# vwxyzjn/cleanrl

Hardware: NVIDIA H100
Metric: env steps/sec (SPS) PPO Breakout num_envs=1024 (higher is better)
Workload: dtype bf16

## Files before the change

cleanrl_b200/_lib.py:

```python
from __future__ import annotations

import ctypes as C
from pathlib import Path

PKG = Path(__file__).resolve().parent
LIB_PATH = PKG / "libb200rl.so"

_p = C.c_void_p
_i64 = C.c_int64
_i = C.c_int
_d = C.c_double
_sz = C.c_size_t

SIGNATURES = {
    "b200rl_version": (_i, []),
    "b200rl_last_error": (C.c_char_p, []),
    "b200rl_compiled_arch": (_i, []),
    "b200rl_launch_count": (C.c_longlong, []),
    "b200rl_profile_enable": (None, [_i]),
    "b200rl_profile_reset": (None, []),
    "b200rl_profile_summary": (_i, [C.c_char_p, _sz]),
    "b200rl_gae_f32": (_i, [_p, _p, _p, _p, _p, _p, _p, _i64, _i64, _d, _d, _i, _p]),
    "b200rl_categorical_sample_f32": (_i, [_p, _i64, _p, _p, _i64, _i64, _i, _p, _p, _p, _p, _p]),
    "b200rl_categorical_eval_f32": (_i, [_p, _i64, _p, _i64, _i, _p, _p, _p]),
    "b200rl_ppo_loss_workspace_bytes": (_sz, [_i64]),
    "b200rl_ppo_loss_f32": (_i, [_p, _i64, _p, _i64, _p, _p, _p, _p, _p, _p, _i64, _i, _d, _d, _d, _i, _i,
                                 _p, _i64, _p, _i64, _p, _p, _sz, _p]),
    "b200rl_gaussian_sample_f32": (_i, [_p, _i64, _p, _p, _p, _i64, _i64, _i, _p, _p, _p, _p, _p]),
    "b200rl_gaussian_eval_f32": (_i, [_p, _i64, _p, _p, _i64, _i, _p, _p, _p]),
    "b200rl_ppo_loss_gaussian_workspace_bytes": (_sz, [_i64]),
    "b200rl_ppo_loss_gaussian_f32": (_i, [_p, _i64, _p, _p, _i64, _p, _p, _p, _p, _p, _p, _i64, _i, _d, _d, _d, _i, _i,
                                          _p, _i64, _p, _p, _i64, _p, _p, _sz, _p]),
    "b200rl_clip_adam_workspace_bytes": (_sz, [_i64]),
    "b200rl_clip_adam_f32": (_i, [_p, _p, _p, _p, _i64, _i64, _d, _d, _d, _d, _d, _i, _p, _p, _sz, _p]),
    "b200rl_adam_step_scalars": (_i, [_i64, _d, _d, _d, _p]),
    "b200rl_clip_adam_dyn_f32": (_i, [_p, _p, _p, _p, _i64, _p, _d, _d, _d, _d, _i, _p, _p, _sz, _p]),
    "b200rl_conv2d_fwd_f32": (_i, [_p, _i, _p, _d, _p, _p, _p, _i64, _i, _i, _i, _i, _i, _i, _i, _i, _p]),
    "b200rl_conv2d_bwd_data_f32": (_i, [_p, _p, _p, _i, _p, _i64, _i, _i, _i, _i, _i, _i, _i, _p]),
    "b200rl_conv2d_bwd_weight_workspace_bytes": (_sz, [_i64, _i, _i, _i, _i, _i, _i, _i]),
    "b200rl_conv2d_bwd_weight_f32": (_i, [_p, _i, _p, _d, _p, _p, _p, _i64, _i, _i, _i, _i, _i, _i, _i, _p, _sz, _p]),
    "b200rl_conv2d_fwd_pad_f32": (_i, [_p, _i, _p, _d, _p, _p, _p, _i64, _i, _i, _i, _i, _i, _i, _i, _i, _i, _p]),
    "b200rl_conv2d_bwd_data_pad_f32": (_i, [_p, _p, _p, _i, _p, _i64, _i, _i, _i, _i, _i, _i, _i, _i, _p]),
    "b200rl_conv2d_bwd_weight_pad_workspace_bytes": (_sz, [_i64, _i, _i, _i, _i, _i, _i, _i, _i]),
    "b200rl_conv2d_bwd_weight_pad_f32": (_i, [_p, _i, _p, _d, _p, _p, _p, _i64, _i, _i, _i, _i, _i, _i, _i, _i, _p, _sz, _p]),
    "b200rl_maxpool3s2_fwd_f32": (_i, [_p, _i64, _i, _i, _p, _p, _p]),
    "b200rl_maxpool3s2_bwd_f32": (_i, [_p, _p, _i64, _i, _i, _p, _p]),
    "b200rl_relu_f32": (_i, [_p, _i64, _p, _p]),
    "b200rl_relu_bwd_f32": (_i, [_p, _p, _p, _i64, _p, _p]),
    "b200rl_add_f32": (_i, [_p, _p, _i64, _p, _p]),
    "b200rl_nhwc_to_nchw_u8": (_i, [_p, _p, _i64, _i, _i, _i, _p, _p]),
    "b200rl_linear_fwd_f32": (_i, [_p, _p, _p, _p, _p, _i64, _i, _i, _i, _p]),
    "b200rl_linear_bwd_data_f32": (_i, [_p, _p, _p, _i, _p, _i64, _i, _i, _p]),
    "b200rl_linear_bwd_weight_workspace_bytes": (_sz, [_i64, _i, _i]),
    "b200rl_linear_bwd_weight_f32": (_i, [_p, _p, _p, _p, _p, _i64, _i, _i, _p, _sz, _p]),
    "b200rl_dqn_td_loss_workspace_bytes": (_sz, [_i64]),
    "b200rl_dqn_td_loss_f32": (_i, [_p, _i64, _p, _i64, _p, _p, _p, _i64, _i, _d, _i, _p, _i64, _p, _p, _sz, _p]),
    "b200rl_argmax_f32": (_i, [_p, _i64, _i64, _i, _p, _p]),
    "b200rl_c51_act_f32": (_i, [_p, _i64, _p, _i64, _i, _i, _p, _p, _p, _p, _p]),
    "b200rl_c51_loss_workspace_bytes": (_sz, [_i64]),
    "b200rl_c51_loss_f32": (_i, [_p, _i64, _p, _i64, _p, _p, _p, _p, _i64, _i, _i, _d, _d, _d, _p, _i64, _p, _p, _sz, _p]),
    "b200rl_naturecnn_param_count": (_i64, [_i]),
    "b200rl_naturecnn_bf16_packed_bytes": (_sz, [_i]),
    "b200rl_naturecnn_bf16_acts_bytes": (_sz, [_i64, _i]),
    "b200rl_frames_to_s2d_bf16": (_i, [_p, _p, _i64, _p, _p]),
    "b200rl_naturecnn_bf16_workspace_bytes": (_sz, [_i64, _i]),
    "b200rl_naturecnn_bf16_pack": (_i, [_p, _i, _p, _p]),
    "b200rl_naturecnn_bf16_forward": (_i, [_p, _i, _p, _i64, _i, _p, _p, _p, _p, _p]),
    "b200rl_naturecnn_bf16_backward": (_i, [_p, _p, _i, _p, _i64, _i, _p, _p, _p, _p, _p, _p, _sz, _p, _p]),
    "b200rl_frames_to_s2d_u8": (_i, [_p, _p, _i64, _p, _p, _p]),
    "b200rl_lstm_mask_state_f32": (_i, [_p, _p, _p, _i64, _i, _p, _p, _p]),
    "b200rl_lstm_cell_fwd_f32": (_i, [_p, _p, _p, _i64, _i, _p, _p, _p, _p]),
    "b200rl_lstm_cell_bwd_f32": (_i, [_p, _p, _p, _p, _p, _p, _p, _i64, _i, _p, _p, _p]),
    "b200rl_naturecnn_grad_tail_offset": (_i64, [_i]),
    "b200rl_frames_delta_s2d_u8": (_i, [_p, _p, _p, _p, _p, _i64, _p, _p, _p]),
    "b200rl_h2d_rows_async": (_i, [_p, _p, _i64, _i64, _i64, _p]),
    "b200rl_stackdelta_create": (_p, [_i64, _i, _i64, _i]),
    "b200rl_stackdelta_destroy": (None, [_p]),
    "b200rl_stackdelta_invalidate": (None, [_p]),
    "b200rl_stackdelta_begin": (_i64, [_p, _p, _i64, _p, _p, _p, _p]),
    "b200rl_stackdelta_wait": (_i64, [_p, _p]),
    "b200rl_mt19937_shuffle_i64": (_i, [_p, _p, _p, _i64]),
    "b200rl_stackdelta_launch": (_i64, [_p, _p, _i64, _p]),
    "b200rl_stackdelta_join": (_i64, [_p, _p, _p]),
    "b200rl_impala_param_count": (_i64, [_i]),
    "b200rl_impala_bf16_packed_bytes": (_sz, [_i]),
    "b200rl_impala_bf16_acts_bytes": (_sz, [_i64]),
    "b200rl_impala_bf16_acts_layout": (_i, [_i64, _p]),
    "b200rl_impala_bf16_workspace_bytes": (_sz, [_i64, _i]),
    "b200rl_impala_bf16_pack": (_i, [_p, _i, _p, _p]),
    "b200rl_impala_bf16_forward": (_i, [_p, _p, _i64, _i, _p, _p, _p, _p, _p]),
    "b200rl_impala_bf16_backward": (_i, [_p, _p, _i64, _i, _p, _p, _p, _p, _p, _p, _sz, _p]),
    "b200rl_impala_ppg_param_count": (_i64, [_i]),
    "b200rl_impala_ppg_bf16_packed_bytes": (_sz, [_i]),
    "b200rl_impala_ppg_bf16_workspace_bytes": (_sz, [_i64, _i]),
    "b200rl_impala_ppg_bf16_pack": (_i, [_p, _i, _p, _p]),
    "b200rl_impala_ppg_bf16_forward": (_i, [_p, _p, _i64, _i, _p, _p, _p, _p, _p]),
    "b200rl_impala_ppg_bf16_backward": (_i, [_p, _p, _i64, _i, _p, _p, _p, _p, _p, _p, _sz, _p]),
    "b200rl_clip_adam_ranges_f32": (_i, [_p, _p, _p, _p, _i64, _i64, _d, _p, _i, _i64, _d, _d, _d, _d, _d, _p, _p, _sz, _p]),
    "b200rl_clip_adam_ranges_dyn_f32": (_i, [_p, _p, _p, _p, _i64, _p, _p, _i, _i, _d, _d, _d, _d, _p, _p, _sz, _p]),
    "b200rl_ppg_aux_loss_workspace_bytes": (_sz, [_i64]),
    "b200rl_ppg_aux_loss_f32": (_i, [_p, _i64, _p, _p, _p, _i64, _i, _d, _d, _p, _i64, _p, _p, _sz, _p]),
    "b200rl_lstm_agent_param_count": (_i64, [_i]),
    "b200rl_lstm_agent_bf16_packed_bytes": (_sz, [_i]),
    "b200rl_lstm_agent_bf16_acts_bytes": (_sz, [_i64, _i64]),
    "b200rl_lstm_agent_bf16_acts_layout": (_i, [_i64, _i64, _p]),
    "b200rl_lstm_agent_bf16_workspace_bytes": (_sz, [_i64, _i64, _i]),
    "b200rl_lstm_agent_bf16_pack": (_i, [_p, _i, _p, _p]),
    "b200rl_lstm_agent_bf16_forward": (_i, [_p, _p, _i64, _i64, _i, _p, _p, _p, _p, _p, _p, _p, _p, _p, _p]),
    "b200rl_lstm_agent_bf16_backward": (_i, [_p, _p, _i64, _i64, _i, _p, _p, _p, _p, _p, _p, _p, _sz, _p]),
}



class PartLaunch(C.Structure):
    _fields_ = [("tracker", _p), ("copy_stream", _p), ("main_stream", _p), ("consumed_event", _p),
                ("n", C.c_int32), ("nchunks", C.c_int32), ("chunk_lo", C.c_int32 * 4), ("chunk_hi", C.c_int32 * 4),
                ("h2d_event", _p * 4), ("graph_exec", _p * 4),
                ("new_d", _p), ("slot_d", _p), ("full_d", _p), ("new_h", _p), ("full_h", _p), ("slot_h", _p),
                ("actions_d", _p), ("actions_h", _p), ("actions_bytes", _i64), ("d2h_event", _p)]


_lib = None


def load():
    global _lib
    if _lib is not None:
        return _lib
    if not LIB_PATH.exists():
        raise RuntimeError(
            f"{LIB_PATH} is missing: build it with `python -m cleanrl_b200.build` "
            "(the CUDA extension is the product; there is no CPU/torch fallback)")
    lib = C.CDLL(str(LIB_PATH))
    for name, (res, args) in SIGNATURES.items():
        fn = getattr(lib, name)
        fn.restype = res
        fn.argtypes = args
    _lib = lib
    return lib


def check(rc, what):
    if rc != 0:
        msg = load().b200rl_last_error().decode("utf-8", "replace")
        raise RuntimeError(f"libb200rl {what} failed (status {rc}): {msg}")
```

cleanrl_b200/agents.py:

```python
from __future__ import annotations

import numpy as np
import torch
import torch.nn as nn

from . import nets, ops


def layer_init(layer, std=np.sqrt(2), bias_const=0.0):
    torch.nn.init.orthogonal_(layer.weight, std)
    torch.nn.init.constant_(layer.bias, bias_const)
    return layer


def _exp_noise(n, A, device):
    return torch.empty(n, A, dtype=torch.float32, device=device).exponential_(1)


_exp_noise.graph_safe = True
_exp_noise.inplace = lambda buf: buf.exponential_(1)


class KernelAgent(nn.Module):

# ... 50 lines not shown

    @property
    def graph_friendly(self):
        return getattr(self.noise_fn, "graph_safe", False) and self.graph_capturable

    def noise_shape(self, n):
        return (n, self.num_actions)

    def draw_noise_into(self, buf):
        if hasattr(self.noise_fn, "inplace"):
            self.noise_fn.inplace(buf)
        else:
            buf.copy_(self.noise_fn(buf.shape[0], buf.shape[1], buf.device))

    def sample_into(self, obs, actions_out, logprobs_out, values_out, noise=None):
        logits, value = self._forward_heads(obs)
        n, A = logits.shape
        q = noise if noise is not None else self.noise_fn(n, A, logits.device)
        ops.categorical_sample(logits, q, value, out=(actions_out, logprobs_out, None, values_out))

    def loss_backward(self, policy_out, value, mb_inds, b, a, stats_row, scratch):
        M = policy_out.shape[0]
        if scratch.get("M") != M:
            scratch["M"] = M
            scratch["dhead"], scratch["dl"], scratch["dv"] = self.alloc_head_grad(M, policy_out.device)
        ops.ppo_loss(policy_out, value, mb_inds, b["actions"], b["logprobs"], b["advantages"], b["returns"], b["values"],
                     a.clip_coef, a.ent_coef, a.vf_coef, a.norm_adv, a.clip_vloss,
                     dlogits=scratch["dl"], dvalue=scratch["dv"], stats=stats_row)
        self.backward(scratch["dhead"])

    def alloc_head_grad(self, M, device):
        A = self.num_actions
        d = torch.empty(M, A + 1, dtype=torch.float32, device=device)
        return d, d[:, :A], d[:, A]

    def get_value(self, x):
        self.flat
        _, value = self._forward_heads(x)
        return value.reshape(-1, 1).clone() if not value.is_contiguous() else value.reshape(-1, 1)

    def get_action_and_value(self, x, action=None):
        self.flat
        logits, value = self._forward_heads(x)
        n, A = logits.shape
        if action is None:
            q = self.noise_fn(n, A, logits.device)
            action, logprob, entropy, v = ops.categorical_sample(logits, q, value)
        else:
            logprob, entropy = ops.categorical_eval(logits, action)
            v = value.clone() if not value.is_contiguous() else value
        return action, logprob, entropy, v.reshape(-1, 1)


class TensorCoreAgent(KernelAgent):

    precision = "fp32"
    plan_class = None
    _tc = None
    _tc_dirty = True

    def _head_outputs(self):
        return self.num_actions + 1

    def _plan_actions(self):
        return self._head_outputs() - 1

    def bind(self):
        self._tc, self._tc_dirty = None, True
        return super().bind()

    def uses_tc_plan(self):
        return self.precision == "bf16"

    @property
    def graph_capturable(self):
        return self.uses_tc_plan()

    def params_updated(self):
        self._tc_dirty = True

    def _tc_plan(self):
        f = self._flat
        if self._tc is None:
            self._tc = self.plan_class(self._plan_actions(), f.flat.device)
            assert f.flat.numel() >= self._tc.param_count
        if self._tc_dirty:
            self._tc.pack(f.flat)
            self._tc_dirty = False
        return self._tc

    def load_state_dict(self, *a, **k):
        out = super().load_state_dict(*a, **k)
        self._tc_dirty = True
        return out

    def pin_workspaces(self):
        if self._tc is not None:
            self._tc.pin()

    def _joint_head(self):
        f, A1, H = self._flat, self._head_outputs(), self.actor.in_features
        ow = (f.view_of(self.actor.weight)[0].data_ptr() - f.flat.data_ptr()) // 4
        ob = (f.view_of(self.actor.bias)[0].data_ptr() - f.flat.data_ptr()) // 4
        return nets.Linear(None, None, f.flat[ow:ow + A1 * H].view(A1, H), f.flat[ob:ob + A1],
                           f.grad[ow:ow + A1 * H].view(A1, H), f.grad[ob:ob + A1])


class NatureCNNAgent(TensorCoreAgent):

    plan_class = ops.NatureCNNBf16

    def __init__(self, envs):
        super().__init__()
        c, h, w = envs.single_observation_space.shape
        assert (c, h, w) == (4, 84, 84), "NatureCNN geometry is 4x84x84"
        trunk = []
        for cin, cout, k, s in ((4, 32, 8, 4), (32, 64, 4, 2), (64, 64, 3, 1)):
            trunk += [layer_init(nn.Conv2d(cin, cout, k, stride=s)), nn.ReLU()]
        trunk += [nn.Flatten(), layer_init(nn.Linear(64 * 7 * 7, 512)), nn.ReLU()]
        self.network = nn.Sequential(*trunk)
        self.actor = layer_init(nn.Linear(512, envs.single_action_space.n), std=0.01)
        self.critic = layer_init(nn.Linear(512, 1), std=1)
        self.num_actions = int(envs.single_action_space.n)

    def _param_order(self):
        net = [p for m in self.network for p in m.parameters()]
        return net + [self.actor.weight, self.critic.weight, self.actor.bias, self.critic.bias]

    def _build_plan(self):
        n = self.network
        self.trunk = nets.Chain([
            nets.Conv(n[0], "relu", in_div=255.0), nets.Conv(n[2], "relu"), nets.Conv(n[4], "relu"),
            nets.Linear(n[7], "relu")])
        self.head = self._joint_head()

    def _forward_heads(self, x, rows=None, keep=False, aux=None):
        if self.precision == "bf16":
            if x.dtype not in (torch.uint8, torch.bfloat16):
                x = x.to(torch.uint8)
            tc = self._tc_plan()
            out = tc.forward(x.contiguous(), rows, self._flat.flat)
            if keep:
                self._tc_obs, self._tc_rows, self._tc_aux = x, rows, aux
            A = self.num_actions
            return out[:, :A], out[:, A]
        if x.dtype not in (torch.uint8, torch.float32):
            x = x.float()
        hidden = self.trunk.fwd(x.contiguous(), rows=rows, keep=keep)
        out = self.head.fwd(hidden)
        if keep:
            self._hidden = hidden
        A = self.num_actions
        return out[:, :A], out[:, A]

    def forward_train(self, b_obs, mb_inds, aux=None):
        self.flat
        return self._forward_heads(b_obs, rows=mb_inds, keep=True, aux=aux)

    def grad_tail(self):
        if self.precision != "bf16":
            return None
        if getattr(self, "_tail_event", None) is None:
            self._tail_event = torch.cuda.Event()
            self._tail_event.record()
        return self._tc_plan().grad_tail_offset(), self._tail_event

    def backward(self, dhead):
        if self.precision == "bf16":
            self._tc.backward(self._tc_obs, self._tc_rows, self._flat.flat, dhead, self._flat.grad,
                              tail_event=getattr(self, "_tail_event", None), obs_aux=getattr(self, "_tc_aux", None))
            self._tc_obs = self._tc_rows = self._tc_aux = None
            return
        hidden = self._hidden
        self.head.bwd_weight(hidden, dhead)
        dh = self.head.bwd_data(dhead, hidden, "relu")
        self.trunk.bwd(dh)
        self._hidden = None


class MLPAgent(KernelAgent):

    def __init__(self, envs):
        super().__init__()
        d = int(np.array(envs.single_observation_space.shape).prod())
        A = int(envs.single_action_space.n)
        self.critic = nn.Sequential(layer_init(nn.Linear(d, 64)), nn.Tanh(), layer_init(nn.Linear(64, 64)), nn.Tanh(),
                                    layer_init(nn.Linear(64, 1), std=1.0))
        self.actor = nn.Sequential(layer_init(nn.Linear(d, 64)), nn.Tanh(), layer_init(nn.Linear(64, 64)), nn.Tanh(),
                                   layer_init(nn.Linear(64, A), std=0.01))
        self.num_actions = A

    def _build_plan(self):
        mk = lambda seq: nets.Chain([nets.Linear(seq[0], "tanh"), nets.Linear(seq[2], "tanh"), nets.Linear(seq[4], None)])
        self.c_chain, self.a_chain = mk(self.critic), mk(self.actor)

    def _forward_heads(self, x, rows=None, keep=False):
        x = x.float() if x.dtype != torch.float32 else x
        x = x.reshape(x.shape[0], -1).contiguous()
        logits = self.a_chain.fwd(x, rows=rows, keep=keep)
        value = self.c_chain.fwd(x, rows=rows, keep=keep)
        return logits, value[:, 0]

    def forward_train(self, b_obs, mb_inds):
        self.flat
        return self._forward_heads(b_obs, rows=mb_inds, keep=True)

    def alloc_head_grad(self, M, device):
        dl = torch.empty(M, self.num_actions, dtype=torch.float32, device=device)
        dv = torch.empty(M, 1, dtype=torch.float32, device=device)
        return (dl, dv), dl, dv[:, 0]

    def backward(self, dhead):
        dl, dv = dhead
        self.a_chain.bwd(dl)
        self.c_chain.bwd(dv)


class LSTMAgent(TensorCoreAgent):

    plan_class = ops.LSTMAgentBf16
    graph_capturable = False

    def __init__(self, envs):
        super().__init__()
        c, h, w = envs.single_observation_space.shape
        assert (h, w) == (84, 84), "NatureCNN trunk geometry is 84x84"
        trunk = []
        for cin, cout, k, s in ((c, 32, 8, 4), (32, 64, 4, 2), (64, 64, 3, 1)):
            trunk += [layer_init(nn.Conv2d(cin, cout, k, stride=s)), nn.ReLU()]
        trunk += [nn.Flatten(), layer_init(nn.Linear(64 * 7 * 7, 512)), nn.ReLU()]
        self.network = nn.Sequential(*trunk)
        self.lstm = nn.LSTM(512, 128)
        for name, param in self.lstm.named_parameters():
            if "bias" in name:
                nn.init.constant_(param, 0)
            elif "weight" in name:
                nn.init.orthogonal_(param, 1.0)
        self.actor = layer_init(nn.Linear(128, envs.single_action_space.n), std=0.01)
        self.critic = layer_init(nn.Linear(128, 1), std=1)
        self.num_actions = int(envs.single_action_space.n)
        self.hidden_size = 128

    def _param_order(self):
        net = [p for m in self.network for p in m.parameters()]
        return net + list(self.lstm.parameters()) + [self.actor.weight, self.critic.weight, self.actor.bias, self.critic.bias]

    def _build_plan(self):
        n = self.network
        self.trunk = nets.Chain([nets.Conv(n[0], "relu", in_div=255.0), nets.Conv(n[2], "relu"), nets.Conv(n[4], "relu"),
                                 nets.Linear(n[7], "relu")])
        self.head = self._joint_head()
        L = self.lstm
        self.l_ih = nets.Linear(None, None, L.weight_ih_l0.data, L.bias_ih_l0.data, L.weight_ih_l0.grad, L.bias_ih_l0.grad)
        self.l_hh = nets.Linear(None, None, L.weight_hh_l0.data, L.bias_hh_l0.data, L.weight_hh_l0.grad, L.bias_hh_l0.grad)

    def _tc_states(self, x, lstm_state, done, rows, keep):
        ops.LSTMAgentBf16.check_obs(x)
        H = self.hidden_size
        h0 = lstm_state[0].reshape(-1, H).to(torch.float32).contiguous()
        c0 = lstm_state[1].reshape(-1, H).to(torch.float32).contiguous()
        n = h0.shape[0]
        total = rows.numel() if rows is not None else x.shape[0]
        assert total % n == 0, "the sequence batch must be steps x envs"
        S = total // n
        done = done.reshape(-1).to(torch.float32).contiguous()
        x = x.contiguous()
        tc = self._tc_plan()
        self._tc_head, h, c = tc.forward(x, rows, S, n, self._flat.flat, h0, c0, done)
        if keep:
            self._tc_seq = (x, rows, S, n, done)
        return tc.act_tensors(S, n)["hseq"], (h.view(1, n, H), c.view(1, n, H))

    def get_states(self, x, lstm_state, done, rows=None, keep=False):
        self.flat
        if self.precision == "bf16":
            return self._tc_states(x, lstm_state, done, rows, keep)
        H = self.hidden_size
        h, c = lstm_state[0].reshape(-1, H).contiguous(), lstm_state[1].reshape(-1, H).contiguous()
        n = h.shape[0]
        if x.dtype not in (torch.uint8, torch.float32):
            x = x.float()
        feats = self.trunk.fwd(x.contiguous(), rows=rows, keep=keep)
        total = feats.shape[0]
        assert total % n == 0, "the sequence batch must be steps x envs"
        S = total // n
        dev = feats.device
        done = done.reshape(S, n).to(torch.float32).contiguous()
        gx = self.l_ih.fwd(feats)
        hidden = torch.empty(S, n, H, dtype=torch.float32, device=dev)
        hm = torch.empty(S, n, H, dtype=torch.float32, device=dev)
        cm = torch.empty(S, n, H, dtype=torch.float32, device=dev)
        save = torch.empty(S, n, 5 * H, dtype=torch.float32, device=dev) if keep else None
        c_cur = torch.empty(n, H, dtype=torch.float32, device=dev)
        for t in range(S):
            ops.lstm_mask_state(h, c, done[t], out=(hm[t], cm[t]))
            gh = self.l_hh.fwd(hm[t])
            ops.lstm_cell_fwd(gx[t * n:(t + 1) * n], gh, cm[t], hidden[t], c_cur, save[t] if keep else None)
            h, c = hidden[t], c_cur
            if t + 1 < S:
                c_cur = torch.empty(n, H, dtype=torch.float32, device=dev)
        if keep:
            self._seq = dict(feats=feats, hidden=hidden, hm=hm, cm=cm, save=save, done=done, S=S, n=n)
        return hidden.view(S * n, H), (h.reshape(1, n, H).clone(), c.reshape(1, n, H).clone())

    def _heads(self, hidden):
        out = self._tc_head if self.precision == "bf16" else self.head.fwd(hidden)
# ... 480 lines not shown
```

cleanrl_b200/csrc/net_tc.cu:

```cuda
#include <cuda.h>
#include <algorithm>
#include "tc_base.cuh"
#include "tc_conv_win.cuh"
#include "tc_conv1_u8.cuh"
#include "tc_gemm_tma.cuh"
#include "tc_wgrad_win.cuh"
#include "tc_reduce.cuh"
#include "tc_aux.cuh"
#include "tc_heads.cuh"
#include "tc_heads_wide.cuh"
#include "tc_lstm.cuh"

namespace b200rl {

struct NatureLayout {
    int A;
    int64_t c1w, c1b, c2w, c2b, c3w, c3b, fcw, fcb, hw, hb, total;
    int64_t w1f, w2f, w2dg, w3f, w3dg, wfcf, wfcdg, w1l, w1sc, packed_total;
    bool wide; int G; int64_t whf, whdg, hbp;
    int64_t wih, whh, bih, bhh, whhp;
    explicit NatureLayout(int A_) : A(A_), wih(-1), whh(-1), bih(-1), bhh(-1), whhp(-1) {
        int64_t o = 0;
        c1w = o; o += 32 * 4 * 8 * 8;  c1b = o; o += 32;
        c2w = o; o += 64 * 32 * 4 * 4; c2b = o; o += 64;
// ... 16 lines not shown
        G = wide ? (int)ceil_div(A + 1, kWideHeadPad) * kWideHeadPad : 0;
        whf = whdg = hbp = 0;
        if (wide) {
            whf = q; q += (int64_t)G * 512;
            whdg = q; q += (int64_t)G * 512;
            hbp = q; q += (int64_t)G * 2;
        }
        packed_total = q;
    }
    struct Lstm {};
    NatureLayout(int A_, Lstm) : A(A_) {
        int64_t o = 0;
        c1w = o; o += 32 * 8 * 8;      c1b = o; o += 32;
        c2w = o; o += 64 * 32 * 4 * 4; c2b = o; o += 64;
        c3w = o; o += 64 * 64 * 3 * 3; c3b = o; o += 64;
        fcw = o; o += 512 * 3136;      fcb = o; o += 512;
        wih = o; o += 512 * 512;       whh = o; o += 512 * 128;
        bih = o; o += 512;             bhh = o; o += 512;
        hw = o;  o += (int64_t)(A + 1) * 128;
        hb = o;  o += A + 1;
        total = o;
        int64_t q = 0;
        w1f = q; q += 32 * 64;
        w2f = q; q += 64 * 512;
        w2dg = q; q += 4 * 32 * 256;
        w3f = q; q += 64 * 576;
        w3dg = q; q += 64 * 576;
        wfcf = q; q += 512 * 3136;
        wfcdg = q; q += 3136 * 512;
        w1l = w1sc = -1;
        wide = true; G = 512;
        whf = q; q += 512 * 512;
        whdg = q; q += 512 * 512;
        hbp = q; q += 512 * 2;
        whhp = q; q += 512 * 128;
        packed_total = q;
    }
};

struct NatureActs {
    int64_t x0, act1, act2, act3, hid, dhid, dact3a, dact3b, dact2a, dact2b, dact1, m1, m2, m3, m4, total;
    explicit NatureActs(int64_t n, bool with_x0 = true) {
        int64_t o = 0;
        x0 = o; if (with_x0) o += n * 28224;
        act1 = o; o += n * 12800;
        act2 = o; o += n * 5184;
        act3 = o; o += n * 3136;
        hid = o;  o += n * 512;
        dhid = o; o += n * 512;
        dact3a = o; o += n * 5184;
        dact3b = o; o += n * 7744;
        dact2a = o; o += n * 6400;
        dact2b = o; o += n * 7744;
        dact1 = o; o += n * 14112;
        auto pad8 = [](int64_t v) { return (v + 7) & ~int64_t(7); };
        m1 = o; o += pad8(n * 100 * 4 * 2);
        m2 = o; o += pad8(n * 81 * 2 * 2);
        m3 = o; o += pad8(n * 49 * 2 * 2);
        m4 = o; o += pad8(n * 16 * 2);
        total = o;
    }
};

static void gemm_rowmajor(KGemmParams& p, const bf16* x, int64_t n, int nchunks) {
    memset(&p, 0, sizeof(p));
    p.scale = 1.f;
    p.A = x; p.M = n; p.nchunks = nchunks;
}


static void win_defaults(WinParams& p) { memset(&p, 0, sizeof(p)); p.scale = 1.f; }
static int round8(int v) { return (v + 7) & ~7; }
static void win_conv1(WinParams& p, const bf16* x0, const int64_t* rows, int64_t n) {
    p.A = x0; p.rows = rows; p.n = (int)n; p.G = 441; p.Wp = 21; p.M = n * 441;
    p.tpi_shift = 2;
    p.n_images = rows ? (int64_t)1 << 24 : n;
    p.ntaps = 4; p.shift[0] = 0; p.shift[1] = 1; p.shift[2] = 21; p.shift[3] = 22; p.WR = round8(128 + 22);
}
static void win_conv2(WinParams& p, const bf16* act1, int64_t n) {
    p.A = act1; p.n = (int)n; p.G = 100; p.Wp = 10; p.M = n * 100;
    p.ntaps = 4; p.shift[0] = 0; p.shift[1] = 1; p.shift[2] = 10; p.shift[3] = 11; p.WR = round8(128 + 11);
}
static void win_conv3(WinParams& p, const bf16* act2, int64_t n) {
    p.A = act2; p.n = (int)n; p.G = 81; p.Wp = 9; p.M = n * 81;
    p.ntaps = 9; for (int ky = 0; ky < 3; ++ky) for (int kx = 0; kx < 3; ++kx) p.shift[ky * 3 + kx] = ky * 9 + kx;
    p.WR = round8(128 + 20);
}
static void wgw_defaults(WGradWinParams& w) { memset(&w, 0, sizeof(w)); }

static const int kC1Ctas = 264, kC2Ctas = 132, kC3Ctas = 132;
static WPlan conv1_wgrad_plan(int64_t n, bool u8) {
    return u8 ? wgrad_plan(n * 512, kC2Ctas, 512) : wgrad_plan(n * 512, kC1Ctas, 128);
}
static WPlan conv2_wgrad_plan(int64_t n) { return wgrad_plan(n * 100, kC2Ctas, 128); }
static WPlan conv3_wgrad_plan(int64_t n) { return wgrad_plan(n * 81, kC3Ctas, 128); }

static size_t wgrad_win_bytes(int splits, int nslots) { return (size_t)splits * nslots * 64 * 64 * sizeof(float); }
static size_t wgrad_win_bias_bytes(int splits) { return (size_t)splits * 64 * sizeof(float); }
static int launch_wgrad_win(const WGradWinParams& p, int ctas, cudaStream_t s, const char* what) {
    const size_t smem = (size_t)kWgradWinStages * ((size_t)p.WRX * 128 * p.cpr + 128 * 128) + 4096 + 1024;
    static SmemAttrCache attr;
    if (int rc0 = attr.ensure(tc_wgrad_win, smem, what)) return rc0;
    CUtensorMap tmX, tmY;
    memset(&tmX, 0, sizeof(tmX)); memset(&tmY, 0, sizeof(tmY));
    const int use_tma = p.tpi_shift ? 0 : 1;
    if (p.rows_per_cta % 128 != 0) return fail(B200RL_ERR_INVALID_ARGUMENT, "%s: rows per CTA must be a multiple of 128", what);
    if (ctas < 1 || (int64_t)(ctas - 1) * p.rows_per_cta >= p.M)
        return fail(B200RL_ERR_INVALID_ARGUMENT, "%s: every row split must own at least one row", what);
    int rc;
    if (use_tma) {
        if (p.rows || p.ldy != 64 || p.ncolsY != 64)
            return fail(B200RL_ERR_INVALID_ARGUMENT, "%s: linear-grid mode needs contiguous rows and 64-channel dY", what);
        if ((rc = make_tmap_2d(&tmX, p.X, p.M, (int64_t)p.cpr * 64, p.WRX, what))) return rc;
        if ((rc = make_tmap_2d(&tmY, p.Y, p.M, 64, 128, what))) return rc;
    } else {
        if ((128 << p.tpi_shift) < p.G) return fail(B200RL_ERR_INVALID_ARGUMENT, "%s: steps per image too small", what);
        if ((rc = make_tmap_3d(&tmX, p.X, p.n_images, p.G, (int64_t)p.cpr * 64, p.WRX, what))) return rc;
    }
    const dim3 grid((unsigned)ceil_div(p.nslots / 2, kWgradWinTilesPerCta), ctas);
    tc_wgrad_win<<<grid, kWgradWinThreads, smem, s>>>(tmX, tmY, p, use_tma);
    return check_launch(what);
}

}

using namespace b200rl;

namespace b200rl {
static bool head_ok(int A) { return A >= 1 && A < kMaxWideHeads; }
static size_t wide_dhead_bytes(int64_t n, const NatureLayout& L) { return ((size_t)n * L.G * 2 + 255) & ~(size_t)255; }
static size_t wide_small_bytes(int64_t n, const NatureLayout& L, int A1) {
    return wide_dhead_bytes(n, L) + colsum_f32_ws(n, A1);
}

static int trunk_fwd(const NatureLayout& L, const NatureActs& Q, const float* params, const bf16* P, bf16* act, int64_t n,
                     cudaStream_t s) {
    int rc;
    KGemmParams p;
    WinParams wp;
    win_defaults(wp); win_conv2(wp, act + Q.act1, n);
    wp.Bw = P + L.w2f; wp.N = 64; wp.vH = 9; wp.vW = 9; wp.out_mode = WOUT_DENSE; wp.out = act + Q.act2;
    wp.bias = params + L.c2b; wp.relu = 1; wp.mask_out = reinterpret_cast<uint32_t*>(act + Q.m2);
    { ProfScope ps(s, "conv2_fwd", 2.0 * n * 81 * 64 * 512, (double)n * ((12800 + 5184) * 2 + 648));
      if ((rc = launch_conv_win_t<128, 2, 2, 4>(wp, s, "naturecnn/conv2"))) return rc; }
    win_defaults(wp); win_conv3(wp, act + Q.act2, n);
    wp.Bw = P + L.w3f; wp.N = 64; wp.vH = 7; wp.vW = 7; wp.out_mode = WOUT_DENSE; wp.out = act + Q.act3;
    wp.bias = params + L.c3b; wp.relu = 1; wp.mask_out = reinterpret_cast<uint32_t*>(act + Q.m3);
    { ProfScope ps(s, "conv3_fwd", 2.0 * n * 49 * 64 * 576, (double)n * ((5184 + 3136) * 2 + 392));
      if ((rc = launch_conv_win_t<128, 1, 4, 9>(wp, s, "naturecnn/conv3"))) return rc; }
    gemm_rowmajor(p, act + Q.act3, n, 49);
    p.Bw = P + L.wfcf; p.N = 512; p.out = act + Q.hid; p.ldo = 512; p.bias = params + L.fcb; p.relu = 1;
    p.mask_out = reinterpret_cast<uint32_t*>(act + Q.m4);
    { ProfScope ps(s, "fc_fwd", 2.0 * n * 512 * 3136, (double)n * (3136 + 512) * 2 + 512.0 * 3136 * 2);
      if (n <= 8192) { if ((rc = launch_gemm_tma<64, 6>(p, s, "naturecnn/fc"))) return rc; }
      else if ((rc = launch_gemm_tma<128, 4>(p, s, "naturecnn/fc"))) return rc; }
    return B200RL_OK;
}

static int trunk_bwd(const NatureLayout& L, const NatureActs& Q, const bf16* P, bf16* act, float* grads, int64_t n,
                     float* wsbig, float* wssmall, void* tail_ready_event, bool dact1_fused, cudaStream_t s) {
    int rc;
    KGemmParams p;
    {
        int splits;
        { ProfScope ps(s, "fc_wgrad", 2.0 * n * 512 * 3136, (double)n * (3136 + 512) * 2 + 512.0 * 3136 * 4);
          if ((splits = launch_wgrad_tma(act + Q.dhid, 512, act + Q.act3, 3136, n, wsbig, s, "naturecnn/fc_wgrad")) < 0) return splits; }
        { ProfScope ps(s, "wgrad_fold_bias", 0, 0);
          note_launches(1); tc_fold_fc<<<(unsigned)ceil_div((int64_t)512 * 3136, 256), 256, 0, s>>>(wsbig, splits, 512, 13 * 256, 512, 3136, 64, 49, 1.f, grads + L.fcw);
          if ((rc = colsum(act + Q.dhid, n, 512, 512, wssmall, grads + L.fcb, s))) return rc; }
        if (tail_ready_event) {
            cudaError_t e = cudaEventRecord(reinterpret_cast<cudaEvent_t>(tail_ready_event), s);
            if (e != cudaSuccess) return fail(B200RL_ERR_CUDA, "naturecnn_backward: cudaEventRecord: %s", cudaGetErrorString(e));
        }
        gemm_rowmajor(p, act + Q.dhid, n, 8);
        p.Bw = P + L.wfcdg; p.N = 3136; p.out = act + Q.dact3a; p.out2 = act + Q.dact3b; p.dual_dact3 = 1;
        p.ldo = 3136; p.mask_bits = reinterpret_cast<const uint32_t*>(act + Q.m3);
        { ProfScope ps(s, "fc_dgrad", 2.0 * n * 512 * 3136, (double)n * ((3136 + 512) * 2 + 392) + 512.0 * 3136 * 2);
          if ((rc = launch_gemm_tma<128, 4>(p, s, "naturecnn/fc_dgrad"))) return rc; }
    }
    WGradWinParams gw;
    WinParams wp;
    FoldWin fw;
    {
        wgw_defaults(gw);
        gw.X = act + Q.act2; gw.M = n * 81; gw.n = (int)n; gw.G = 81; gw.cpr = 1; gw.nslots = 10; gw.WRX = round8(128 + 20);
        for (int t = 0; t < 9; ++t) gw.shift[t] = (t / 3) * 9 + (t % 3);
        const int st[10] = {0, 1, 2, 3, 4, 5, 6, 7, 7, 8};
        for (int k = 0; k < 10; ++k) { gw.slot_tap[k] = st[k]; gw.slot_cc[k] = 0; }
        gw.Y = act + Q.dact3a; gw.ldy = 64; gw.ncolsY = 64;
        const WPlan pl = conv3_wgrad_plan(n);
        gw.rows_per_cta = pl.rows_per_cta; gw.ws = wsbig; gw.wsb = wssmall;
        { ProfScope ps(s, "conv3_wgrad", 2.0 * n * 49 * 64 * 576, (double)n * (5184 + 5184) * 2);
          if ((rc = launch_wgrad_win(gw, pl.splits, s, "naturecnn/conv3_wgrad"))) return rc; }
        memset(&fw, 0, sizeof(fw));
        fw.layer = 3; fw.S = pl.splits; fw.nslots = 10; fw.Cout = 64; fw.scale = 1.f; fw.bscale = 1.f;
        for (int k = 0; k < 10; ++k) { fw.slot_tap[k] = st[k]; fw.slot_skip[k] = (k == 8); }
        { ProfScope ps(s, "wgrad_fold_bias", 0, 0);
          fw.wsb = wssmall; fw.db = grads + L.c3b;
          tc_fold_win<<<(unsigned)ceil_div(640 * 64 + 64, 32), 256, 0, s>>>(wsbig, fw, grads + L.c3w);
          if ((rc = check_launch("naturecnn/conv3_fold"))) return rc; }
        win_defaults(wp);
        wp.A = act + Q.dact3b; wp.n = (int)n; wp.G = 121; wp.Wp = 11; wp.M = n * 121; wp.ntaps = 9;
        for (int ky = 0; ky < 3; ++ky) for (int kx = 0; kx < 3; ++kx) wp.shift[ky * 3 + kx] = (2 - ky) * 11 + (2 - kx);
        wp.WR = round8(128 + 24);
        wp.Bw = P + L.w3dg; wp.N = 64; wp.vH = 9; wp.vW = 9; wp.out_mode = WOUT_DACT2;
        wp.out = act + Q.dact2a; wp.out2 = act + Q.dact2b; wp.mask_bits = reinterpret_cast<const uint32_t*>(act + Q.m2);
        { ProfScope ps(s, "conv3_dgrad", 2.0 * n * 81 * 64 * 576, (double)n * ((7744 + 6400 + 7744) * 2 + 648));
          if ((rc = launch_conv_win_t<128, 1, 4, 9>(wp, s, "naturecnn/conv3_dgrad"))) return rc; }
    }
    {
        wgw_defaults(gw);
        gw.X = act + Q.act1; gw.M = n * 100; gw.n = (int)n; gw.G = 100; gw.cpr = 2; gw.nslots = 8; gw.WRX = round8(128 + 11);
        gw.shift[0] = 0; gw.shift[1] = 1; gw.shift[2] = 10; gw.shift[3] = 11;
        for (int k = 0; k < 8; ++k) { gw.slot_tap[k] = k >> 1; gw.slot_cc[k] = k & 1; }
        gw.Y = act + Q.dact2a; gw.ldy = 64; gw.ncolsY = 64;
        const WPlan pl = conv2_wgrad_plan(n);
        gw.rows_per_cta = pl.rows_per_cta; gw.ws = wsbig; gw.wsb = wssmall;
        { ProfScope ps(s, "conv2_wgrad", 2.0 * n * 81 * 64 * 512, (double)n * (12800 + 6400) * 2);
          if ((rc = launch_wgrad_win(gw, pl.splits, s, "naturecnn/conv2_wgrad"))) return rc; }
        memset(&fw, 0, sizeof(fw));
        fw.layer = 2; fw.S = pl.splits; fw.nslots = 8; fw.Cout = 64; fw.scale = 1.f; fw.bscale = 1.f;
        for (int k = 0; k < 8; ++k) { fw.slot_tap[k] = k >> 1; fw.slot_cc[k] = k & 1; }
        { ProfScope ps(s, "wgrad_fold_bias", 0, 0);
          fw.wsb = wssmall; fw.db = grads + L.c2b;
          tc_fold_win<<<(unsigned)ceil_div(512 * 64 + 64, 32), 256, 0, s>>>(wsbig, fw, grads + L.c2w);
          if ((rc = check_launch("naturecnn/conv2_fold"))) return rc; }
        if (dact1_fused) return B200RL_OK;
        win_defaults(wp);
        wp.A = act + Q.dact2b; wp.n = (int)n; wp.G = 121; wp.Wp = 11; wp.M = n * 121; wp.ntaps = 4;
        for (int a = 0; a < 2; ++a) for (int b = 0; b < 2; ++b) wp.shift[a * 2 + b] = (1 - a) * 11 + (1 - b);
        wp.WR = round8(128 + 12);
        wp.Bw = P + L.w2dg; wp.N = 128; wp.vH = 10; wp.vW = 10; wp.out_mode = WOUT_DACT1;
        wp.out = act + Q.dact1; wp.mask_bits = reinterpret_cast<const uint32_t*>(act + Q.m1);
        { ProfScope ps(s, "conv2_dgrad", 2.0 * n * 400 * 32 * 256, (double)n * ((7744 + 14112) * 2 + 1600));
          if ((rc = launch_conv_win<128, 1, 4, 4>(wp, s, "naturecnn/conv2_dgrad"))) return rc; }
    }
    return B200RL_OK;
}
static size_t trunk_big_bytes(int64_t n) {
    return std::max({wgrad_tma_bytes(n, 512, 3136), wgrad_win_bytes(conv3_wgrad_plan(n).splits, 10),
                     wgrad_win_bytes(conv2_wgrad_plan(n).splits, 8)});
}
static size_t trunk_small_bytes(int64_t n) {
    return std::max({colsum_ws(n, 512), wgrad_win_bias_bytes(conv3_wgrad_plan(n).splits),
                     wgrad_win_bias_bytes(conv2_wgrad_plan(n).splits)});
}

static int wide_head_fwd(const NatureLayout& L, const bf16* P, const bf16* hid, int64_t n, int A1, float* out, cudaStream_t s) {
    KGemmParams p;
    gemm_rowmajor(p, hid, n, 8);
    p.Bw = P + L.whf; p.N = L.G; p.bias = reinterpret_cast<const float*>(P + L.hbp);
    p.out_f32 = out; p.ldo = A1; p.ncols_f32 = A1;
    return launch_gemm_tma<128, 4>(p, s, "wide_heads");
}

static int wide_head_bwd(const NatureLayout& L, const bf16* P, const float* dhead, int64_t n, int A1, const bf16* hid, bf16* dhid,
                         const uint32_t* hid_bits, float* dW, float* db, float* wsbig, float* wssmall, cudaStream_t s) {
    int rc;
    KGemmParams p;
    bf16* dh16 = reinterpret_cast<bf16*>(wssmall);
    float* dbpart = reinterpret_cast<float*>(reinterpret_cast<char*>(wssmall) + wide_dhead_bytes(n, L));
    int cb = (int)ceil_div(n * L.G, 256); if (cb > num_sms() * 8) cb = num_sms() * 8;
    tc_head_dhead_bf16<<<cb, 256, 0, s>>>(dhead, n, A1, L.G, dh16);
    if ((rc = check_launch("wide_heads_dhead"))) return rc;
    if ((rc = colsum_f32(dhead, n, A1, dbpart, db, s))) return rc;
    const int splits = launch_wgrad_tma(dh16, L.G, hid, 512, n, wsbig, s, "wide_heads_wgrad");
    if (splits < 0) return splits;
    tc_fold_fc<<<(unsigned)ceil_div((int64_t)A1 * 512, 256), 256, 0, s>>>(wsbig, splits, L.G, 512, A1, 512, 512, 1, 1.f, dW);
    if ((rc = check_launch("wide_heads_wgrad"))) return rc;
    gemm_rowmajor(p, dh16, n, L.G / 64);
    p.Bw = P + L.whdg; p.N = 512; p.out = dhid; p.ldo = 512;
    p.mask_bits = hid_bits;
    if (n <= 8192) { if ((rc = launch_gemm_tma<64, 6>(p, s, "wide_heads_dgrad"))) return rc; }
    else if ((rc = launch_gemm_tma<128, 4>(p, s, "wide_heads_dgrad"))) return rc;
    return B200RL_OK;
}
}

extern "C" int64_t b200rl_naturecnn_param_count(int A) { return A >= 1 ? NatureLayout(A).total : -1; }
extern "C" int64_t b200rl_naturecnn_grad_tail_offset(int A) { return A >= 1 ? NatureLayout(A).fcw : -1; }
extern "C" size_t b200rl_naturecnn_bf16_packed_bytes(int A) { return head_ok(A) ? (size_t)NatureLayout(A).packed_total * 2 : 0; }
extern "C" size_t b200rl_naturecnn_bf16_acts_bytes(int64_t n, int obs_format) {
    return n >= 0 ? (size_t)NatureActs(n, obs_format == B200RL_OBS_U8_NCHW).total * 2 + 256 : 0;
}

extern "C" int b200rl_frames_to_s2d_bf16(const uint8_t* obs, const int64_t* rows, int64_t n, void* out, void* stream) {
    B200RL_REQUIRE(n >= 0, "frames_to_s2d: negative n");
    if (n == 0) return B200RL_OK;
    B200RL_REQUIRE(obs && out, "frames_to_s2d: null pointer");
    B200RL_REQUIRE(aligned(obs, 4) && aligned(out, 16), "frames_to_s2d: misaligned buffer");
    cudaStream_t s = (cudaStream_t)stream;
    ProfScope ps(s, "frames_to_s2d", 0, (double)n * 28224 * 3);
    tc_frames_to_s2d<<<(unsigned)ceil_div(n * 1764, 256), 256, 0, s>>>(obs, rows, n, reinterpret_cast<bf16*>(out));
    return check_launch("frames_to_s2d");
}

extern "C" int b200rl_frames_to_s2d_u8(const uint8_t* obs, const int64_t* rows, int64_t n, uint8_t* out_rm, uint8_t* out_cm, void* stream) {
    B200RL_REQUIRE(n >= 0, "frames_to_s2d_u8: negative n");
    if (n == 0) return B200RL_OK;
    B200RL_REQUIRE(obs && out_rm && out_cm, "frames_to_s2d_u8: null pointer");
    B200RL_REQUIRE(aligned(obs, 16) && aligned(out_rm, 16) && aligned(out_cm, 16), "frames_to_s2d_u8: misaligned buffer");
    B200RL_REQUIRE(n <= (int64_t)1 << 28, "frames_to_s2d_u8: n too large");
    cudaStream_t s = (cudaStream_t)stream;
    ProfScope ps(s, "frames_to_s2d", 0, (double)n * (28224 + 28224 + 28672));
    tc_frames_to_s2d_u8<<<(unsigned)(n * 4), 256, 0, s>>>(obs, rows, n, out_rm, out_cm);
    return check_launch("frames_to_s2d_u8");
}

static size_t naturecnn_big_bytes(int64_t n, const NatureLayout& L) {
    return std::max({trunk_big_bytes(n), L.wide ? wgrad_tma_bytes(n, L.G, 512) : 0,
                     wgrad_win_bytes(conv1_wgrad_plan(n, false).splits, 4), wgrad_win_bytes(conv1_wgrad_plan(n, true).splits, 4)});
}

extern "C" size_t b200rl_naturecnn_bf16_workspace_bytes(int64_t n, int A) {
    if (n < 1 || !head_ok(A)) return 0;
    const NatureLayout L(A);
    const size_t small = std::max({trunk_small_bytes(n), L.wide ? wide_small_bytes(n, L, A + 1) : heads_partial_bytes(n, A + 1, 512),
                                   wgrad_win_bias_bytes(conv1_wgrad_plan(n, false).splits),
                                   wgrad_win_bias_bytes(conv1_wgrad_plan(n, true).splits)});
    return naturecnn_big_bytes(n, L) + small + 512;
}

extern "C" int b200rl_naturecnn_bf16_pack(const float* params, int A, void* packed, void* stream) {
    B200RL_REQUIRE(params && packed && head_ok(A), "naturecnn_pack: bad arguments (A must be in [1,%d])", kMaxWideHeads - 1);
    B200RL_REQUIRE(aligned(packed, 16), "naturecnn_pack: packed buffer must be 16-B aligned");
    const NatureLayout L(A);
    bf16* P = reinterpret_cast<bf16*>(packed);
    cudaStream_t s = (cudaStream_t)stream;
    ProfScope ps(s, "pack_weights", 0, (double)L.total * 4 + (double)L.packed_total * 2);
    tc_pack_conv1_s2d<<<32, 256, 0, s>>>(params + L.c1w, P + L.w1f);
    tc_pack_conv1_i8<<<32, 256, 0, s>>>(params + L.c1w, reinterpret_cast<int8_t*>(P + L.w1l), reinterpret_cast<float*>(P + L.w1sc));
    tc_pack_conv2_cells<<<128, 256, 0, s>>>(params + L.c2w, P + L.w2f);
    tc_pack_conv_s2_classes<<<(unsigned)ceil_div(32768, 256), 256, 0, s>>>(params + L.c2w, 64, 32, P + L.w2dg);
    tc_pack_conv<<<(unsigned)ceil_div(36864, 256), 256, 0, s>>>(params + L.c3w, 64, 64, 3, 3, 0, P + L.w3f, P + L.w3dg);
    tc_pack_fc<<<dim3(512 / 8, 49 / 7), 256, 0, s>>>(params + L.fcw, 512, 49, P + L.wfcf, P + L.wfcdg);
    if (L.wide) {
        tc_pack_head_wide<<<(unsigned)ceil_div((int64_t)L.G * 512, 256), 256, 0, s>>>(params + L.hw, params + L.hb, A + 1, L.G,
                                                                                    P + L.whf, P + L.whdg, reinterpret_cast<float*>(P + L.hbp));
        return check_launch("naturecnn_pack", 7);
    }
    return check_launch("naturecnn_pack", 6);
}

extern "C" int b200rl_naturecnn_bf16_forward(const void* obs, int obs_format, const int64_t* rows, int64_t n, int A,
                                             const float* params, const void* packed, void* acts,
                                             float* head_out, void* stream) {
    B200RL_REQUIRE(n >= 0, "naturecnn_forward: negative n");
    if (n == 0) return B200RL_OK;
    B200RL_REQUIRE(obs && params && packed && acts && head_out, "naturecnn_forward: null pointer");
    B200RL_REQUIRE(head_ok(A), "naturecnn_forward: A=%d outside [1,%d]", A, kMaxWideHeads - 1);
    B200RL_REQUIRE(obs_format == B200RL_OBS_U8_NCHW || obs_format == B200RL_OBS_S2D_BF16 || obs_format == B200RL_OBS_S2D_U8,
                   "naturecnn_forward: bad obs_format %d", obs_format);
    B200RL_REQUIRE(aligned(obs, 16) && aligned(acts, 16) && aligned(packed, 16), "naturecnn_forward: misaligned buffer");
    B200RL_REQUIRE(n <= (int64_t)1 << 22, "naturecnn_forward: n too large");
    const NatureLayout L(A);
    const NatureActs Q(n, obs_format == B200RL_OBS_U8_NCHW);
    const bf16* P = reinterpret_cast<const bf16*>(packed);
    bf16* act = reinterpret_cast<bf16*>(acts);
    cudaStream_t s = (cudaStream_t)stream;
    int rc;
    WinParams wp;
    const bf16* x0 = reinterpret_cast<const bf16*>(obs);
    const int64_t* x0rows = rows;
    if (obs_format == B200RL_OBS_U8_NCHW) {
        if ((rc = b200rl_frames_to_s2d_bf16(reinterpret_cast<const uint8_t*>(obs), rows, n, act + Q.x0, stream))) return rc;
        x0 = act + Q.x0; x0rows = nullptr;
    }
    if (obs_format == B200RL_OBS_S2D_U8) {
        Conv1U8Params cp;
        memset(&cp, 0, sizeof(cp));
        cp.rows = rows; cp.n = (int)n; cp.n_images = rows ? (int64_t)1 << 24 : n;
        cp.limbs = reinterpret_cast<const int8_t*>(P + L.w1l); cp.sc = reinterpret_cast<const float*>(P + L.w1sc);
        cp.bias = params + L.c1b; cp.out = act + Q.act1; cp.mask_out = reinterpret_cast<uint32_t*>(act + Q.m1);
        ProfScope ps(s, "conv1_fwd", 2.0 * n * 400 * 32 * 256, (double)n * (28224 + 12800 * 2 + 1600));
        if ((rc = launch_conv1_i8(cp, obs, s, "naturecnn/conv1_i8"))) return rc;
    } else {
    win_defaults(wp); win_conv1(wp, x0, x0rows, n);
    wp.Bw = P + L.w1f; wp.N = 32; wp.vH = 20; wp.vW = 20; wp.out_mode = WOUT_S2D2; wp.out = act + Q.act1;
    wp.bias = params + L.c1b; wp.scale = 1.0f / 255.0f; wp.relu = 1; wp.mask_out = reinterpret_cast<uint32_t*>(act + Q.m1);
    { ProfScope ps(s, "conv1_fwd", 2.0 * n * 400 * 32 * 256, (double)n * ((28224 + 12800) * 2 + 1600));
      if ((rc = launch_conv_win<32, 1, 9, 4>(wp, s, "naturecnn/conv1"))) return rc; }
    }
    if ((rc = trunk_fwd(L, Q, params, P, act, n, s))) return rc;
    if (L.wide) {
        ProfScope ps(s, "heads_fwd", 2.0 * n * 512 * (A + 1), (double)n * (1024 + 4 * (A + 1)) + (double)L.G * 1024);
        return wide_head_fwd(L, P, act + Q.hid, n, A + 1, head_out, s);
    }
    ProfScope ps(s, "heads_fwd", 2.0 * n * 512 * (A + 1), (double)n * (1024 + 4 * (A + 1)));
    return heads_fwd<512>(act + Q.hid, params + L.hw, params + L.hb, n, A + 1, head_out, s, "naturecnn/heads");
}

extern "C" int b200rl_naturecnn_bf16_backward(const void* obs, const void* obs_aux, int obs_format, const int64_t* rows, int64_t n, int A,
                                              const float* params, const void* packed, void* acts,
                                              const float* dhead, float* grads,
                                              void* workspace, size_t workspace_bytes, void* tail_ready_event, void* stream) {
    B200RL_REQUIRE(n >= 1, "naturecnn_backward: n must be >= 1");
    B200RL_REQUIRE(obs && params && packed && acts && dhead && grads && workspace, "naturecnn_backward: null pointer");
    B200RL_REQUIRE(head_ok(A), "naturecnn_backward: A=%d outside [1,%d]", A, kMaxWideHeads - 1);
    B200RL_REQUIRE(aligned(workspace, 16), "naturecnn_backward: workspace misaligned");
    const size_t need = b200rl_naturecnn_bf16_workspace_bytes(n, A);
    if (workspace_bytes < need) return fail(B200RL_ERR_WORKSPACE, "naturecnn_backward: workspace %zu < %zu", workspace_bytes, need);
    B200RL_REQUIRE(obs_format == B200RL_OBS_U8_NCHW || obs_format == B200RL_OBS_S2D_BF16 || obs_format == B200RL_OBS_S2D_U8,
                   "naturecnn_backward: bad obs_format %d", obs_format);
    B200RL_REQUIRE(obs_format != B200RL_OBS_S2D_U8 || (obs_aux && aligned(obs_aux, 16)), "naturecnn_backward: the uint8 rollout needs obs_aux");
    const NatureLayout L(A);
    const NatureActs Q(n, obs_format == B200RL_OBS_U8_NCHW);
    const bf16* P = reinterpret_cast<const bf16*>(packed);
    bf16* act = reinterpret_cast<bf16*>(acts);
    cudaStream_t s = (cudaStream_t)stream;
    const bf16* x0 = obs_format == B200RL_OBS_U8_NCHW ? act + Q.x0 : reinterpret_cast<const bf16*>(obs);
    const int64_t* x0rows = obs_format == B200RL_OBS_U8_NCHW ? nullptr : rows;
    const size_t big = (naturecnn_big_bytes(n, L) + 255) & ~(size_t)255;
    float* wsbig = reinterpret_cast<float*>(workspace);
    float* wssmall = reinterpret_cast<float*>(reinterpret_cast<char*>(workspace) + big);
    int rc;
    const int A1 = A + 1;
    if (L.wide) {
        ProfScope ps(s, "heads_bwd", 4.0 * n * 512 * A1, (double)n * (2048 + 64 + 8 * A1));
        if ((rc = wide_head_bwd(L, P, dhead, n, A1, act + Q.hid, act + Q.dhid, reinterpret_cast<const uint32_t*>(act + Q.m4),
                                grads + L.hw, grads + L.hb, wsbig, wssmall, s))) return rc;
    } else
    {
        ProfScope ps(s, "heads_bwd", 4.0 * n * 512 * A1, (double)n * (2048 + 64 + 8 * A1));
        if ((rc = heads_bwd_weight<512>(dhead, act + Q.hid, n, A1, wssmall, grads + L.hw, grads + L.hb, s, "naturecnn/heads_bwd"))) return rc;
        if ((rc = heads_bwd_data<512>(dhead, params + L.hw, reinterpret_cast<const uint8_t*>(act + Q.m4), n, A1, act + Q.dhid, s,
                                      "naturecnn/heads_bwd"))) return rc;
    }
    if ((rc = trunk_bwd(L, Q, P, act, grads, n, wsbig, wssmall, tail_ready_event, obs_format == B200RL_OBS_S2D_U8, s))) return rc;
    const bool u8 = obs_format == B200RL_OBS_S2D_U8;
    const WPlan pl = conv1_wgrad_plan(n, u8);
    if (u8) {
        Conv21BwdU8Params cw;
        memset(&cw, 0, sizeof(cw));
        cw.rows = rows; cw.n = (int)n; cw.rows_per_cta = pl.rows_per_cta; cw.ws = wsbig; cw.wsb = wssmall;
        cw.w2dg = P + L.w2dg; cw.m1 = reinterpret_cast<const uint32_t*>(act + Q.m1);
        { ProfScope ps(s, "conv21_bwd", 2.0 * 2.0 * n * 400 * 32 * 256, (double)n * (7744 * 2 + 1600 + 28672 + 14112 * 2));
          if ((rc = launch_conv21_bwd_u8(cw, obs_aux, rows ? (int64_t)1 << 24 : n, act + Q.dact2b, act + Q.dact1, pl.splits, s,
                                         "naturecnn/conv21_bwd_u8"))) return rc; }
    } else {
        WGradWinParams gw;
        wgw_defaults(gw);
        gw.X = x0; gw.rows = x0rows; gw.M = n * 512; gw.n = (int)n; gw.G = 441; gw.cpr = 1; gw.nslots = 4; gw.WRX = round8(128 + 22);
        gw.tpi_shift = 2; gw.n_images = x0rows ? (int64_t)1 << 24 : n;
        gw.shift[0] = 0; gw.shift[1] = 1; gw.shift[2] = 21; gw.shift[3] = 22;
        for (int k = 0; k < 4; ++k) { gw.slot_tap[k] = k; gw.slot_cc[k] = 0; }
        gw.Y = act + Q.dact1; gw.ldy = 32; gw.ncolsY = 32;
        gw.rows_per_cta = pl.rows_per_cta; gw.ws = wsbig; gw.wsb = wssmall;
        { ProfScope ps(s, "conv1_wgrad", 2.0 * n * 400 * 32 * 256, (double)n * (28224 + 14112) * 2);
          if ((rc = launch_wgrad_win(gw, pl.splits, s, "naturecnn/conv1_wgrad"))) return rc; }
    }
    FoldWin fw;
    memset(&fw, 0, sizeof(fw));
    fw.layer = 1; fw.S = pl.splits; fw.nslots = 4; fw.Cout = 32;
    fw.scale = u8 ? 1.0f / 255.0f / kDact1Scale : 1.0f / 255.0f;
    fw.bscale = u8 ? 1.0f / kDact1Scale : 1.f;
    for (int k = 0; k < 4; ++k) fw.slot_tap[k] = k;
    { ProfScope ps(s, "wgrad_fold_bias", 0, 0);
      fw.wsb = wssmall; fw.db = grads + L.c1b;
      tc_fold_win<<<(unsigned)ceil_div(256 * 32 + 32, 32), 256, 0, s>>>(wsbig, fw, grads + L.c1w);
      if ((rc = check_launch("naturecnn/conv1_fold"))) return rc; }
    return B200RL_OK;
}

namespace b200rl {
constexpr int64_t kLstmMaxRows = (int64_t)1 << 17;

struct LstmActs {
    NatureActs T;
    int64_t gx, hseq, hm, save, cm, dgates, total;
    explicit LstmActs(int64_t M) : T(M, false) {
        int64_t o = (T.total * 2 + 255) & ~int64_t(255);
        auto take = [&](int64_t bytes) { const int64_t r = o; o += (bytes + 255) & ~int64_t(255); return r; };
        gx = take(M * 512 * 4);
        hseq = take(M * 128 * 2);
        hm = take(M * 128 * 2);
        save = take(M * 640 * 4);
        cm = take(M * 128 * 4);
        dgates = take(M * 512 * 4);
        total = o;
    }
};

static bool lstm_heads_ok(int A) { return A >= 1 && A + 1 <= lstm::kMaxA1; }
static bool lstm_sizes_ok(int64_t S, int64_t n) { return S >= 1 && n >= 1 && S <= kLstmMaxRows && n <= kLstmMaxRows && S * n <= kLstmMaxRows; }

struct C1Plan { int64_t per_cta; int ctas; };
static C1Plan lstm_conv1_plan(int64_t M) {
    C1Plan c;
    const int64_t want = M < kC1Ctas ? M : kC1Ctas;
    c.per_cta = ceil_div(M, want);
    c.ctas = (int)ceil_div(M, c.per_cta);
    return c;
}
static size_t lstm_big_bytes(int64_t M, const NatureLayout& L) {
    const size_t a = std::max({wgrad_tma_bytes(M, L.G, 512), wgrad_tma_bytes(M, 512, 128), trunk_big_bytes(M),
                               (size_t)lstm_conv1_plan(M).ctas * 32 * 64 * 4});
    return (a + 255) & ~(size_t)255;
}
static size_t lstm_small_bytes(int64_t M, const NatureLayout& L) {
    return std::max({heads_partial_bytes(M, L.A + 1, 128), wide_small_bytes(M, L, 512), trunk_small_bytes(M),
                     (size_t)lstm_conv1_plan(M).ctas * 32 * 4});
}
}

extern "C" int64_t b200rl_lstm_agent_param_count(int A) { return A >= 1 ? NatureLayout(A, NatureLayout::Lstm{}).total : -1; }
extern "C" size_t b200rl_lstm_agent_bf16_packed_bytes(int A) {
    return lstm_heads_ok(A) ? (size_t)NatureLayout(A, NatureLayout::Lstm{}).packed_total * 2 : 0;
}
extern "C" size_t b200rl_lstm_agent_bf16_acts_bytes(int64_t S, int64_t n) {
    return lstm_sizes_ok(S, n) ? (size_t)LstmActs(S * n).total : 0;
}
extern "C" int b200rl_lstm_agent_bf16_acts_layout(int64_t S, int64_t n, int64_t* offsets) {
    B200RL_REQUIRE(offsets, "lstm_acts_layout: null pointer");
    B200RL_REQUIRE(lstm_sizes_ok(S, n), "lstm_acts_layout: S=%lld n=%lld out of range", (long long)S, (long long)n);
    const LstmActs Q(S * n);
    const int64_t v[B200RL_LSTM_ACTS_TENSORS] = {Q.T.act1 * 2, Q.T.m1 * 2, Q.T.act2 * 2, Q.T.act3 * 2, Q.T.hid * 2, Q.T.m4 * 2,
                                                 Q.gx, Q.hseq, Q.hm, Q.save, Q.cm, Q.dgates, Q.T.dhid * 2};
    for (int k = 0; k < B200RL_LSTM_ACTS_TENSORS; ++k) offsets[k] = v[k];
    return B200RL_OK;
}
extern "C" size_t b200rl_lstm_agent_bf16_workspace_bytes(int64_t S, int64_t n, int A) {
    if (!lstm_sizes_ok(S, n) || !lstm_heads_ok(A)) return 0;
    const NatureLayout L(A, NatureLayout::Lstm{});
    return lstm_big_bytes(S * n, L) + lstm_small_bytes(S * n, L) + 512;
}

extern "C" int b200rl_lstm_agent_bf16_pack(const float* params, int A, void* packed, void* stream) {
    B200RL_REQUIRE(params && packed, "lstm_pack: null pointer");
    B200RL_REQUIRE(lstm_heads_ok(A), "lstm_pack: A=%d outside [1,%d]", A, lstm::kMaxA1 - 1);
    B200RL_REQUIRE(aligned(params, 16) && aligned(packed, 16), "lstm_pack: misaligned buffer");
    const NatureLayout L(A, NatureLayout::Lstm{});
    bf16* P = reinterpret_cast<bf16*>(packed);
    cudaStream_t s = (cudaStream_t)stream;
    ProfScope ps(s, "pack_weights", 0, (double)L.total * 4 + (double)L.packed_total * 2);
    lstm::lstm_pack_conv1<<<8, 256, 0, s>>>(params + L.c1w, P + L.w1f);
    tc_pack_conv2_cells<<<128, 256, 0, s>>>(params + L.c2w, P + L.w2f);
    tc_pack_conv_s2_classes<<<(unsigned)ceil_div(32768, 256), 256, 0, s>>>(params + L.c2w, 64, 32, P + L.w2dg);
    tc_pack_conv<<<(unsigned)ceil_div(36864, 256), 256, 0, s>>>(params + L.c3w, 64, 64, 3, 3, 0, P + L.w3f, P + L.w3dg);
    tc_pack_fc<<<dim3(512 / 8, 49 / 7), 256, 0, s>>>(params + L.fcw, 512, 49, P + L.wfcf, P + L.wfcdg);
    tc_pack_head_wide<<<(unsigned)ceil_div((int64_t)L.G * 512, 256), 256, 0, s>>>(params + L.wih, params + L.bih, 512, L.G,
                                                                                P + L.whf, P + L.whdg, reinterpret_cast<float*>(P + L.hbp));
    tc_head_dhead_bf16<<<256, 256, 0, s>>>(params + L.whh, 512, 128, 128, P + L.whhp);
// ... 122 lines not shown
```

cleanrl_b200/csrc/policy.cu:

```cuda
#include "common.cuh"
#include <cfloat>

namespace b200rl {

constexpr int kMaxA = 64;

struct RowStats {
    float lse;
    float m2;
    float s2;
};

__device__ __forceinline__ RowStats row_stats(const float* __restrict__ x, int A) {
    float m = -INFINITY;
    for (int k = 0; k < A; ++k) m = fmaxf(m, x[k]);
    const float mm = (fabsf(m) == INFINITY) ? 0.f : m;
    float s = 0.f;
    for (int k = 0; k < A; ++k) s += expf(x[k] - mm);
    RowStats r;
    r.lse = logf(s) + mm;
    float m2 = -INFINITY;
    for (int k = 0; k < A; ++k) m2 = fmaxf(m2, x[k] - r.lse);
    float s2 = 0.f;
    for (int k = 0; k < A; ++k) s2 += expf((x[k] - r.lse) - m2);
    r.m2 = m2;
    r.s2 = s2;
    return r;
}

__global__ void __launch_bounds__(128) categorical_sample_kernel(
    const float* __restrict__ logits, int64_t ld, const float* __restrict__ noise,
    const float* __restrict__ value_in, int64_t ldv, int64_t n, int A,
    int64_t* __restrict__ action, float* __restrict__ logprob, float* __restrict__ entropy,
    float* __restrict__ value_out) {
    const int64_t i = (int64_t)blockIdx.x * blockDim.x + threadIdx.x;
    if (i >= n) return;
    const float* x = logits + i * ld;
    const float* q = noise + i * (int64_t)A;
    const RowStats rs = row_stats(x, A);
    float best = -INFINITY, ent = 0.f;
    int arg = 0;
    for (int k = 0; k < A; ++k) {
        const float nl = x[k] - rs.lse;
        const float p = expf(nl - rs.m2) / rs.s2;
        const float sc = p / q[k];
        if (sc > best) { best = sc; arg = k; }
        ent += fmaxf(nl, -FLT_MAX) * p;
    }
    action[i] = arg;
    logprob[i] = x[arg] - rs.lse;
    if (entropy) entropy[i] = -ent;
    if (value_out && value_in) value_out[i] = value_in[i * ldv];
}

__global__ void __launch_bounds__(128) categorical_eval_kernel(
    const float* __restrict__ logits, int64_t ld, const int64_t* __restrict__ action, int64_t n, int A,
    float* __restrict__ logprob, float* __restrict__ entropy) {
    const int64_t i = (int64_t)blockIdx.x * blockDim.x + threadIdx.x;
    if (i >= n) return;
    const float* x = logits + i * ld;
    const RowStats rs = row_stats(x, A);
    float ent = 0.f;
    for (int k = 0; k < A; ++k) {
        const float nl = x[k] - rs.lse;
        ent += fmaxf(nl, -FLT_MAX) * (expf(nl - rs.m2) / rs.s2);
    }
    int a = (int)action[i];
    a = a < 0 ? 0 : (a >= A ? A - 1 : a);
    logprob[i] = x[a] - rs.lse;
    if (entropy) entropy[i] = -ent;
}

__device__ __forceinline__ float adv_pass(const float* __restrict__ b_adv, const int64_t* __restrict__ inds, int64_t M,
                                          float mean, bool squared) {
    float s = 0.f;
    const int64_t step = blockDim.x;
    int64_t i = threadIdx.x;
    for (; i + 7 * step < M; i += 8 * step) {
        int64_t j[8];
        float v[8];
#pragma unroll
        for (int u = 0; u < 8; ++u) j[u] = inds ? __ldg(inds + i + u * step) : i + u * step;
#pragma unroll
        for (int u = 0; u < 8; ++u) v[u] = __ldg(b_adv + j[u]);
#pragma unroll
        for (int u = 0; u < 8; ++u) {
            const float d = v[u] - mean;
            s += squared ? d * d : v[u];
        }
    }
    for (; i < M; i += step) {
        const float v = b_adv[inds ? inds[i] : i];
        const float d = v - mean;
        s += squared ? d * d : v;
    }
    return s;
}
__global__ void __launch_bounds__(1024) adv_stats_kernel(
    const float* __restrict__ b_adv, const int64_t* __restrict__ inds, int64_t M, float* __restrict__ out2) {
    __shared__ float red[32];
    const float mean = block_sum(adv_pass(b_adv, inds, M, 0.f, false), red) / (float)M;
    const float ss = block_sum(adv_pass(b_adv, inds, M, mean, true), red);
    if (threadIdx.x == 0) {
        out2[0] = mean;
        out2[1] = sqrtf(ss / (float)(M - 1));
    }
}

constexpr int kLossThreads = 256;
constexpr int kNumStats = 7;

struct LossParams {
    const float* logits; int64_t ld;
    const float* value; int64_t ldv;
    const int64_t* inds;
    const int64_t* b_actions;
    const float* b_logprobs; const float* b_adv; const float* b_ret; const float* b_val;
    int64_t M; int A;
    float clip, ent_coef, vf_coef;
    int norm_adv, clip_vloss;
    float* dlogits; int64_t ldd;
    float* dvalue; int64_t lddv;
    float* stats;
    const float* adv_stats;
    float* partials;
    unsigned int* ticket;
};

__global__ void __launch_bounds__(kLossThreads) ppo_loss_kernel(LossParams P) {
    __shared__ float red[32];
    __shared__ bool is_last;
    const int64_t i = (int64_t)blockIdx.x * blockDim.x + threadIdx.x;
    float acc[kNumStats];
#pragma unroll
    for (int k = 0; k < kNumStats; ++k) acc[k] = 0.f;
    if (i < P.M) {
        const int64_t j = P.inds ? P.inds[i] : i;
        const float* x = P.logits + i * P.ld;
        const int A = P.A;
        const int a = (int)P.b_actions[j];
        const RowStats rs = row_stats(x, A);
        float ent = 0.f;
        for (int k = 0; k < A; ++k) {
            const float nl = x[k] - rs.lse;
            const float p = expf(nl - rs.m2) / rs.s2;
            ent += fmaxf(nl, -FLT_MAX) * p;
        }
        ent = -ent;
        const float newlogprob = x[a] - rs.lse;
        const float logratio = newlogprob - P.b_logprobs[j];
        const float ratio = expf(logratio);
        float adv = P.b_adv[j];
        if (P.norm_adv) adv = (adv - P.adv_stats[0]) / (P.adv_stats[1] + 1e-8f);
        const float lo = 1.f - P.clip, hi = 1.f + P.clip;
        const float rc = fminf(fmaxf(ratio, lo), hi);
        const float pg1 = -adv * ratio, pg2 = -adv * rc;
        const float pg = fmaxf(pg1, pg2);
        const float nv = P.value[i * P.ldv];
        const float R = P.b_ret[j], V = P.b_val[j];
        float vterm, gv;
        const float du = nv - R;
        const float vu = du * du;
        if (P.clip_vloss) {
            const float d = nv - V;
            const float vcl = V + fminf(fmaxf(d, -P.clip), P.clip);
            const float dc = vcl - R;
            const float vc = dc * dc;
            vterm = fmaxf(vu, vc);
            const float gu = 2.f * du;
            const float gc = (d >= -P.clip && d <= P.clip) ? 2.f * dc : 0.f;
            gv = (vu > vc) ? gu : ((vc > vu) ? gc : 0.5f * (gu + gc));
        } else {
            vterm = vu;
            gv = 2.f * du;
        }
        acc[0] = pg;
        acc[1] = vterm;
        acc[2] = ent;
        acc[3] = -logratio;
        acc[4] = (ratio - 1.f) - logratio;
        acc[5] = (fabsf(ratio - 1.0f) > P.clip) ? 1.f : 0.f;
        const float invM = 1.0f / (float)P.M;
        const float inrange = (ratio >= lo && ratio <= hi) ? 1.f : 0.f;
        float g_ratio = 0.f;
        if (pg1 > pg2) g_ratio = -adv;
        else if (pg1 == pg2) g_ratio = 0.5f * (-adv) * (1.f + inrange);
        const float g_lp = g_ratio * ratio * invM;
        const float g_ent = -P.ent_coef * invM;
        float* dl = P.dlogits + i * P.ldd;
        for (int k = 0; k < A; ++k) {
            const float nl = x[k] - rs.lse;
            const float p = expf(nl - rs.m2) / rs.s2;
            const float onehot = (k == a) ? 1.f : 0.f;
            dl[k] = g_lp * (onehot - p) + g_ent * (-p * (nl + ent));
        }
        P.dvalue[i * P.lddv] = P.vf_coef * 0.5f * invM * gv;
    }
#pragma unroll
    for (int k = 0; k < 6; ++k) {
        const float s = block_sum(acc[k], red);
        if (threadIdx.x == 0) P.partials[(int64_t)blockIdx.x * kNumStats + k] = s;
    }
    if (threadIdx.x == 0) {
        __threadfence();
// ... 364 lines not shown
```

cleanrl_b200/csrc/tc_conv1_u8.cuh:

```cuda
#pragma once
#include "tc_base.cuh"
#include <cuda_fp16.h>
#include "tc_conv_win.cuh"

namespace b200rl {
using namespace tc;

__device__ __forceinline__ uint64_t desc_kmajor_sw64(uint32_t smem_addr) {
    return (uint64_t)((smem_addr & 0x3FFFFu) >> 4) | (1ull << 16) | (32ull << 32) | kDescSwizzle64;
}
__device__ __forceinline__ uint64_t desc_mnmajor_sw64(uint32_t smem_addr, uint32_t lbo) {
    return (uint64_t)((smem_addr & 0x3FFFFu) >> 4) | ((uint64_t)((lbo >> 4) & 0x3FFF) << 16) | (32ull << 32) | kDescSwizzle64;
}
__device__ __forceinline__ uint32_t img64_off(int r, int c) { return (uint32_t)(r * 64 + ((c ^ ((r >> 1) & 3)) << 4)); }
__global__ void __launch_bounds__(256) tc_frames_to_s2d_u8(const uint8_t* __restrict__ obs, const int64_t* __restrict__ rows, int64_t n,
                                                           uint8_t* __restrict__ out_rm, uint8_t* __restrict__ out_cm) {
    __shared__ __align__(16) uint8_t plane[7056];
    const int64_t i = blockIdx.x >> 2;
    const int c = blockIdx.x & 3;
    const int64_t img = rows ? rows[i] : i;
    const int4* src = reinterpret_cast<const int4*>(obs + img * 28224 + c * 7056);
    for (int t = threadIdx.x; t < 441; t += 256) reinterpret_cast<int4*>(plane)[t] = __ldg(src + t);
    __syncthreads();
    for (int pos = threadIdx.x; pos < 441; pos += 256) {
        const int Y = pos / 21, X = pos - Y * 21;
        const uint8_t* p = plane + (Y * 4) * 84 + X * 4;
        int4 v;
        v.x = *reinterpret_cast<const int*>(p); v.y = *reinterpret_cast<const int*>(p + 84);
        v.z = *reinterpret_cast<const int*>(p + 168); v.w = *reinterpret_cast<const int*>(p + 252);
        *reinterpret_cast<int4*>(out_rm + (i * 441 + pos) * 64 + c * 16) = v;
    }
    for (int t = threadIdx.x; t < 16 * 112; t += 256) {
        const int ch = t / 112, q = t - ch * 112;
        const int sy = ch >> 2, sx = ch & 3;
        uint32_t w = 0;
#pragma unroll
        for (int e = 0; e < 4; ++e) {
            const int pos = q * 4 + e;
            if (pos < 441) {
                const int Y = pos / 21, X = pos - Y * 21;
                w |= (uint32_t)plane[(Y * 4 + sy) * 84 + X * 4 + sx] << (8 * e);
            }
        }
        *reinterpret_cast<uint32_t*>(out_cm + (i * 64 + c * 16 + ch) * 448 + q * 4) = w;
    }
}

__global__ void __launch_bounds__(256) tc_pack_conv1_i8(const float* __restrict__ w, int8_t* __restrict__ limbs, float* __restrict__ sc) {
    __shared__ float red[32];
    const int co = blockIdx.x, idx = threadIdx.x;
    const float v = w[co * 256 + idx];
    float m = fabsf(v);
#pragma unroll
    for (int o = 16; o > 0; o >>= 1) m = fmaxf(m, __shfl_xor_sync(0xffffffffu, m, o));
    if ((idx & 31) == 0) red[idx >> 5] = m;
    __syncthreads();
    float mx = red[0];
#pragma unroll
    for (int k = 1; k < 8; ++k) mx = fmaxf(mx, red[k]);
    const float s = mx > 0.f ? mx * (128.0f / 127.0f) : 1.0f;
    const float u = v / s * 128.0f;
    float l1 = rintf(u);
    l1 = fminf(fmaxf(l1, -127.f), 127.f);
    float l2 = rintf((u - l1) * 128.0f);
    l2 = fminf(fmaxf(l2, -127.f), 127.f);
    const int kx = idx & 7, ky = (idx >> 3) & 7, c = idx >> 6;
    const int a = ky >> 2, sy = ky & 3, b = kx >> 2, sx = kx & 3;
    const int k = (a * 2 + b) * 64 + c * 16 + sy * 4 + sx;
    limbs[co * 256 + k] = (int8_t)l1;
    limbs[(32 + co) * 256 + k] = (int8_t)l2;
    if (idx == 0) {
        sc[co] = s / 128.0f / 255.0f;
        sc[32 + co] = s / 16384.0f / 255.0f;
    }
}

struct Conv1U8Params {
    const int64_t* rows;
    int n;
    int64_t n_images;
    const int8_t* limbs;
    const float* sc;
    const float* bias;
    bf16* out;
    uint32_t* mask_out;
};

constexpr int kConv1I8Threads = 384;
template <int STAGES>
__global__ void __launch_bounds__(kConv1I8Threads, 1) tc_conv1_i8(const __grid_constant__ CUtensorMap tmA, const Conv1U8Params p, int total_tiles) {
    constexpr int BN = 64, WR = 144, NTAPS = 4;
    constexpr int STAGE_BYTES = WR * 128;
    constexpr int B_CHUNK = BN * 64;
    extern __shared__ uint8_t smem_raw[];
    __shared__ uint64_t full_bar[STAGES], empty_bar[STAGES];
    __shared__ __align__(16) float s_sc[32], s_bias[32];
    uint8_t* smem = reinterpret_cast<uint8_t*>((reinterpret_cast<uintptr_t>(smem_raw) + 1023) & ~uintptr_t(1023));
    const int tid = threadIdx.x, warp = tid >> 5;
    uint8_t* sW = smem;
    uint8_t* sRing = smem + NTAPS * B_CHUNK;

    if (tid == 0) {
        for (int s = 0; s < STAGES; ++s) { mbar_init(&full_bar[s], 1); mbar_init(&empty_bar[s], 8); }
        fence_barrier_init();
        tma_prefetch_desc(&tmA);
    }
    for (int idx = tid; idx < NTAPS * BN * 4; idx += blockDim.x) {
        const int c16 = idx & 3;
        const int t = (idx >> 2) & 3;
        const int r = idx >> 4;
        *reinterpret_cast<int4*>(sW + t * B_CHUNK + img64_off(r, c16)) = ldg16(p.limbs + r * 256 + t * 64 + c16 * 16);
    }
    if (tid < 32) { s_sc[tid] = p.sc[32 + tid]; s_bias[tid] = p.bias[tid]; }
    fence_proxy_async_smem();
    __syncthreads();
    const int tile_begin = (int)(((int64_t)total_tiles * blockIdx.x) / gridDim.x);
    const int tile_end = (int)(((int64_t)total_tiles * (blockIdx.x + 1)) / gridDim.x);

    if (warp == 0) {
        if (tid == 0) {
            uint32_t q = 0;
            int z_next = 0;
            if (tile_begin < tile_end) {
                const int img = tile_begin >> 1;
                z_next = p.rows ? (int)__ldg(p.rows + img) : img;
            }
            for (int tile = tile_begin; tile < tile_end; ++tile, ++q) {
                const uint32_t s = q % STAGES;
                const int z = z_next;
                if (tile + 1 < tile_end) {
                    const int img = (tile + 1) >> 1;
                    z_next = p.rows ? (int)__ldg(p.rows + img) : img;
                }
                if (q >= (uint32_t)STAGES) mbar_wait(&empty_bar[s], ((q / STAGES) - 1) & 1);
                mbar_arrive_expect_tx(&full_bar[s], (uint32_t)STAGE_BYTES);
                tma_load_3d(smem_u32(sRing + (size_t)s * STAGE_BYTES), &tmA, 0, (tile & 1) * 128, z, &full_bar[s]);
            }
        }
    } else if (warp >= 4) {
        const int wg = (warp - 4) >> 2, wt = tid & 127, lane = tid & 31, qd = lane & 3;
        const uint32_t w_base = smem_u32(sW);
        constexpr int off[4] = {0, 1, 21, 22};
        int acc[2][32];
#pragma unroll
        for (int e = 0; e < 2; ++e)
#pragma unroll
            for (int c = 0; c < 32; ++c) acc[e][c] = 0;
        for (int tile = tile_begin; tile < tile_end; ++tile) {
            const uint32_t q = (uint32_t)(tile - tile_begin), s = q % STAGES;
            mbar_wait(&full_bar[s], (q / STAGES) & 1);
            wgmma_fence();
            const uint32_t win = smem_u32(sRing + (size_t)s * STAGE_BYTES) + (uint32_t)(wg * 64 * 128);
#pragma unroll
            for (int e = 0; e < 2; ++e) {
#pragma unroll
                for (int t = 0; t < NTAPS; ++t) {
                    const int po = e + off[t];
                    const uint64_t a = desc_kmajor(win + (uint32_t)((po >> 1) * 128 + (po & 1) * 64));
                    const uint64_t b = desc_kmajor_sw64(w_base + (uint32_t)(t * B_CHUNK));
#pragma unroll
                    for (int kk = 0; kk < 2; ++kk) wgmma_u8s8_n64(acc[e], a + 2 * kk, b + 2 * kk, (t | kk) != 0 ? 1u : 0u);
                }
            }
            wgmma_commit();
            wgmma_wait<0>();
            wgmma_fence_operands(acc[0]);
            wgmma_fence_operands(acc[1]);
            if (lane == 0) mbar_arrive(&empty_bar[s]);
            const int i = tile >> 1;
#pragma unroll
            for (int e = 0; e < 2; ++e) {
#pragma unroll
                for (int hr = 0; hr < 2; ++hr) {
                    const int lrow = wg * 64 + ((wt >> 5) << 4) + (lane >> 2) + 8 * hr;
                    const int rem = 2 * (((tile & 1) << 7) + lrow) + e;
                    const int Y = (rem * 3121) >> 16, X = rem - Y * 21;
                    const bool valid = rem < 441 && Y < 20 && X < 20;
                    const int64_t cell = ((int64_t)i * 10 + (Y >> 1)) * 10 + (X >> 1);
                    const int cls = (Y & 1) * 2 + (X & 1);
                    uint32_t bits = 0u, pk[4];
#pragma unroll
                    for (int j = 0; j < 4; ++j) {
                        const int co = 8 * j + 2 * qd;
                        const float f0 = fmaf((float)(acc[e][4 * j + 2 * hr] * 128 + acc[e][4 * (j + 4) + 2 * hr]), s_sc[co], s_bias[co]);
                        const float f1 = fmaf((float)(acc[e][4 * j + 2 * hr + 1] * 128 + acc[e][4 * (j + 4) + 2 * hr + 1]), s_sc[co + 1],
                                              s_bias[co + 1]);
                        bits |= (f0 > 0.f ? 1u : 0u) << co;
                        bits |= (f1 > 0.f ? 1u : 0u) << (co + 1);
                        pk[j] = pack_bf16x2_relu(f0, f1);
                    }
                    bits |= __shfl_xor_sync(0xffffffffu, bits, 1);
                    bits |= __shfl_xor_sync(0xffffffffu, bits, 2);
                    if (valid) {
                        if (qd == 0) p.mask_out[cell * 4 + cls] = bits;
                        uint32_t* dst = reinterpret_cast<uint32_t*>(reinterpret_cast<uint8_t*>(p.out) + (cell * 4 + cls) * 64);
#pragma unroll
                        for (int j = 0; j < 4; ++j) dst[4 * j + qd] = pk[j];
// ... 319 lines not shown
```

cleanrl_b200/csrc/tc_gemm_tma.cuh:

```cuda
#pragma once
#include "tc_base.cuh"

namespace b200rl {
using namespace tc;

struct KGemmParams {
    const void* A;
    int64_t M;
    int nchunks;
    const bf16* Bw;
    int N;
    bf16* out;
    int ldo;
    const float* bias;
    float scale;
    int relu;
    const uint32_t* mask_bits;
    uint32_t* mask_out;
    int dual_dact3;
    bf16* out2;
    float* out_f32;
    int ncols_f32;
};

constexpr int kGemmThreads = 384;
template <int BN>
__host__ __device__ constexpr size_t gemm_acc_bytes() { return (size_t)128 * (BN + 4) * sizeof(float); }
template <int BN, int STAGES>
__global__ void __launch_bounds__(kGemmThreads, 1) tc_gemm_tma(const __grid_constant__ CUtensorMap tmA,
                                                               const __grid_constant__ CUtensorMap tmB,
                                                               const KGemmParams p, int total_tiles, int ntiles_n) {
    constexpr int A_BYTES = 128 * 128;
    constexpr int B_BYTES = BN * 128;
    constexpr int STAGE_BYTES = A_BYTES + B_BYTES;
    constexpr int LDA = BN + 4;
    extern __shared__ uint8_t smem_raw[];
    __shared__ uint64_t full_bar[STAGES], empty_bar[STAGES];
    uint8_t* smem = reinterpret_cast<uint8_t*>((reinterpret_cast<uintptr_t>(smem_raw) + 1023) & ~uintptr_t(1023));
    float* sAcc = reinterpret_cast<float*>(smem + (size_t)STAGES * STAGE_BYTES);
    const int tid = threadIdx.x, warp = tid >> 5;
    const int nch = p.nchunks;
    if (tid == 0) {
        for (int s = 0; s < STAGES; ++s) { mbar_init(&full_bar[s], 1); mbar_init(&empty_bar[s], 256); }
        fence_barrier_init();
        tma_prefetch_desc(&tmA);
        tma_prefetch_desc(&tmB);
    }
    __syncthreads();

    if (warp == 0) {
        if ((tid & 31) == 0) {
            uint32_t q = 0;
            for (int tile = blockIdx.x; tile < total_tiles; tile += gridDim.x) {
                const int mt = tile / ntiles_n, n0 = (tile - mt * ntiles_n) * BN;
                for (int j = 0; j < nch; ++j, ++q) {
                    const uint32_t s = q % STAGES;
                    if (q >= (uint32_t)STAGES) mbar_wait(&empty_bar[s], ((q / STAGES) - 1) & 1);
                    const uint32_t dst = smem_u32(smem + (size_t)s * STAGE_BYTES);
                    mbar_arrive_expect_tx(&full_bar[s], STAGE_BYTES);
                    tma_load_2d(dst, &tmA, j * 64, mt * 128, &full_bar[s]);
                    tma_load_2d(dst + A_BYTES, &tmB, j * 64, n0, &full_bar[s]);
                }
            }
        }
    } else if (warp >= 4) {
        const int wg = (warp - 4) >> 2, wt = tid & 127;
        float* st = sAcc + wg * 64 * LDA;
        const int lr = wt & 63, half = wt >> 6;
        const int nwords = p.N >> 5;
        constexpr int NW = BN / 32;
        float d[BN / 2];
#pragma unroll
        for (int e = 0; e < BN / 2; ++e) d[e] = 0.f;
        uint32_t q = 0;
        for (int tile = blockIdx.x; tile < total_tiles; tile += gridDim.x) {
            const int mt = tile / ntiles_n, n0 = (tile - mt * ntiles_n) * BN;
            for (int j = 0; j < nch; ++j, ++q) {
                const uint32_t s = q % STAGES;
                mbar_wait(&full_bar[s], (q / STAGES) & 1);
                wgmma_fence();
                const uint32_t stage_addr = smem_u32(smem + (size_t)s * STAGE_BYTES);
                const uint64_t a = desc_kmajor(stage_addr + wg * 64 * 128), b = desc_kmajor(stage_addr + A_BYTES);
#pragma unroll
                for (int kk = 0; kk < 4; ++kk) WgmmaBf16<BN, 0, 0>::mma(d, a + 2 * kk, b + 2 * kk, (j | kk) != 0 ? 1u : 0u);
                wgmma_commit();
                wgmma_wait<0>();
                mbar_arrive(&empty_bar[s]);
            }
            wgmma_fence_operands(d);
            const int r = mt * 128 + wg * 64 + lr;
            const bool rvalid = r < (int)p.M;
            const int64_t wb = (int64_t)r * nwords + (n0 >> 5);
            named_bar(1 + wg, 128);
            stage_acc(st, LDA, wt, d);
            named_bar(1 + wg, 128);
#pragma unroll
            for (int g = 0; g < NW; ++g) {
                const int col = n0 + g * 32;
                if (!rvalid || (g & 1) != half || col >= p.N) continue;
                uint32_t v[32];
#pragma unroll
                for (int e = 0; e < 8; ++e) {
                    const float4 f = *reinterpret_cast<const float4*>(st + lr * LDA + g * 32 + 4 * e);
                    v[4 * e] = __float_as_uint(f.x); v[4 * e + 1] = __float_as_uint(f.y);
                    v[4 * e + 2] = __float_as_uint(f.z); v[4 * e + 3] = __float_as_uint(f.w);
                }
                const uint32_t mbw = p.mask_bits != nullptr ? __ldg(p.mask_bits + wb + g) : 0xFFFFFFFFu;
                if (p.bias) {
                    const float4* bp = reinterpret_cast<const float4*>(p.bias + col);
#pragma unroll
                    for (int e = 0; e < 8; ++e) {
                        const float4 bv = __ldg(bp + e);
                        v[4 * e] = __float_as_uint(fmaf(__uint_as_float(v[4 * e]), p.scale, bv.x));
                        v[4 * e + 1] = __float_as_uint(fmaf(__uint_as_float(v[4 * e + 1]), p.scale, bv.y));
                        v[4 * e + 2] = __float_as_uint(fmaf(__uint_as_float(v[4 * e + 2]), p.scale, bv.z));
                        v[4 * e + 3] = __float_as_uint(fmaf(__uint_as_float(v[4 * e + 3]), p.scale, bv.w));
                    }
                } else {
#pragma unroll
                    for (int e = 0; e < 32; ++e) v[e] = __float_as_uint(__uint_as_float(v[e]) * p.scale);
                }
                if (p.relu) {
                    uint32_t bits = 0u;
#pragma unroll
                    for (int e = 0; e < 32; ++e) {
                        const bool pos = __uint_as_float(v[e]) > 0.f;
                        bits |= (pos ? 1u : 0u) << e;
                        v[e] = pos ? v[e] : 0u;
                    }
                    if (p.mask_out) p.mask_out[wb + g] = bits;
                }
                if (p.mask_bits) {
#pragma unroll
                    for (int e = 0; e < 32; ++e) if (!((mbw >> e) & 1u)) v[e] = 0u;
                }
                if (p.out_f32) {
                    float* dst = p.out_f32 + (int64_t)r * p.ldo + col;
#pragma unroll
                    for (int e = 0; e < 32; ++e) if (col + e < p.ncols_f32) dst[e] = __uint_as_float(v[e]);
                    continue;
                }
                int4 w[4];
#pragma unroll
                for (int e = 0; e < 4; ++e) {
                    w[e].x = (int)pack_bf16x2(__uint_as_float(v[8 * e]), __uint_as_float(v[8 * e + 1]));
                    w[e].y = (int)pack_bf16x2(__uint_as_float(v[8 * e + 2]), __uint_as_float(v[8 * e + 3]));
                    w[e].z = (int)pack_bf16x2(__uint_as_float(v[8 * e + 4]), __uint_as_float(v[8 * e + 5]));
                    w[e].w = (int)pack_bf16x2(__uint_as_float(v[8 * e + 6]), __uint_as_float(v[8 * e + 7]));
                }
                if (p.dual_dact3) {
                    const int px = col >> 6;
                    const int oy = px / 7, ox = px - oy * 7;
                    bf16* dst = p.out + ((int64_t)r * 81 + oy * 9 + ox) * 64 + (g & 1) * 32;
                    bf16* dst2 = p.out2 + ((int64_t)r * 121 + (oy + 2) * 11 + ox + 2) * 64 + (g & 1) * 32;
                    st_global_32b(dst, w[0], w[1]); st_global_32b(dst + 16, w[2], w[3]);
                    st_global_32b(dst2, w[0], w[1]); st_global_32b(dst2 + 16, w[2], w[3]);
                } else {
                    bf16* dst = p.out + (int64_t)r * p.ldo + col;
                    st_global_32b(dst, w[0], w[1]); st_global_32b(dst + 16, w[2], w[3]);
                }
            }
        }
    }
}

constexpr int kWgradTmaThreads = 384;
constexpr int kFcWgradXChunks = 2, kFcWgradYChunks = 4;
static __global__ void __launch_bounds__(kWgradTmaThreads, 1) tc_wgrad_tma(const __grid_constant__ CUtensorMap tmX,
                                                                    const __grid_constant__ CUtensorMap tmY,
                                                                    int64_t M, int64_t rows_per_cta, float* ws) {
    constexpr int R = 64, STAGES = 4, nxc = kFcWgradXChunks, nyc = kFcWgradYChunks, NY = 64 * nyc;
    extern __shared__ uint8_t smem_raw[];
    __shared__ uint64_t full_bar[STAGES], empty_bar[STAGES];
    uint8_t* smem = reinterpret_cast<uint8_t*>((reinterpret_cast<uintptr_t>(smem_raw) + 1023) & ~uintptr_t(1023));
    const int tid = threadIdx.x, warp = tid >> 5;
    const int xc0 = blockIdx.y * nxc, yc0 = blockIdx.z * nyc;
    constexpr int chunk_img = R * 128;
    constexpr int stage_bytes = (nxc + nyc) * chunk_img;
    if (tid == 0) {
        for (int s = 0; s < STAGES; ++s) { mbar_init(&full_bar[s], 1); mbar_init(&empty_bar[s], 8); }
        fence_barrier_init();
        tma_prefetch_desc(&tmX);
        tma_prefetch_desc(&tmY);
    }
    __syncthreads();
    const int64_t m_begin = (int64_t)blockIdx.x * rows_per_cta;
    int64_t m_end = m_begin + rows_per_cta;
    if (m_end > M) m_end = M;
    const int nsteps = m_end > m_begin ? (int)((m_end - m_begin + R - 1) / R) : 0;

    if (warp == 0 && (tid & 31) == 0) {
        for (int it = 0; it < nsteps; ++it) {
            const int s = it % STAGES;
            if (it >= STAGES) mbar_wait(&empty_bar[s], ((it / STAGES) - 1) & 1);
            const uint32_t dst = smem_u32(smem + (size_t)s * stage_bytes);
            const int m0 = (int)(m_begin + (int64_t)it * R);
            mbar_arrive_expect_tx(&full_bar[s], (uint32_t)stage_bytes);
            for (int c = 0; c < nxc; ++c) tma_load_2d(dst + c * chunk_img, &tmX, (xc0 + c) * 64, m0, &full_bar[s]);
            for (int c = 0; c < nyc; ++c) tma_load_2d(dst + (nxc + c) * chunk_img, &tmY, (yc0 + c) * 64, m0, &full_bar[s]);
        }
    } else if (warp >= 4) {
        const int wg = (warp - 4) >> 2, wt = tid & 127;
        float d[NY / 2];
#pragma unroll
        for (int e = 0; e < NY / 2; ++e) d[e] = 0.f;
        for (int it = 0; it < nsteps; ++it) {
            const int s = it % STAGES;
            mbar_wait(&full_bar[s], (it / STAGES) & 1);
            wgmma_fence();
            const uint32_t xa = smem_u32(smem + (size_t)s * stage_bytes), ya = xa + nxc * chunk_img;
#pragma unroll
            for (int kk = 0; kk < R / 16; ++kk) {
                const uint64_t adesc = desc_mnmajor(xa + wg * chunk_img + kk * 2048, chunk_img);
                const uint64_t bdesc = desc_mnmajor(ya + kk * 2048, chunk_img);
                WgmmaBf16<NY, 1, 1>::mma(d, adesc, bdesc, (it | kk) != 0 ? 1u : 0u);
            }
            wgmma_commit();
            wgmma_wait<0>();
            if ((tid & 31) == 0) mbar_arrive(&empty_bar[s]);
        }
        wgmma_fence_operands(d);
        const int64_t NYtot = (int64_t)gridDim.z * nyc * 64;
        const int64_t KXtot = (int64_t)gridDim.y * nxc * 64;
        float* wsb = ws + (int64_t)blockIdx.x * KXtot * NYtot;
        const int row = ((wt >> 5) << 4) + ((wt & 31) >> 2), col = (wt & 3) * 2;
        float* d0 = wsb + ((int64_t)xc0 * 64 + wg * 64 + row) * NYtot + (int64_t)yc0 * 64 + col;
        float* d8 = d0 + 8 * NYtot;
#pragma unroll
        for (int j = 0; j < NY / 8; ++j) {
            *reinterpret_cast<float2*>(d0 + 8 * j) = make_float2(d[4 * j], d[4 * j + 1]);
            *reinterpret_cast<float2*>(d8 + 8 * j) = make_float2(d[4 * j + 2], d[4 * j + 3]);
        }
    }
}

template <int BN, int STAGES>
static int launch_gemm_tma(const KGemmParams& p, cudaStream_t s, const char* what) {
    const size_t smem = (size_t)STAGES * (128 * 128 + BN * 128) + gemm_acc_bytes<BN>() + 1024;
    static SmemAttrCache attr;
    int rc;
    if (p.N % 64 != 0 || BN % 64 != 0) return fail(B200RL_ERR_INVALID_ARGUMENT, "%s: N must be a multiple of 64", what);
    if ((rc = attr.ensure(tc_gemm_tma<BN, STAGES>, smem, what))) return rc;
    CUtensorMap tmA, tmB;
    const int64_t K = (int64_t)p.nchunks * 64;
    if ((rc = make_tmap_2d(&tmA, p.A, p.M, K, 128, what))) return rc;
    if ((rc = make_tmap_2d(&tmB, p.Bw, p.N, K, BN, what))) return rc;
    const int ntn = (int)ceil_div(p.N, BN);
    const int total = (int)ceil_div(p.M, 128) * ntn;
    int grid = num_sms();
    if (grid > total) grid = total;
    tc_gemm_tma<BN, STAGES><<<grid, kGemmThreads, smem, s>>>(tmA, tmB, p, total, ntn);
    return check_launch(what);
}

static int64_t round_up(int64_t a, int64_t b) { return ceil_div(a, b) * b; }
struct WPlan { int64_t rows_per_cta; int splits; };
static WPlan wgrad_plan(int64_t M, int target_ctas, int quantum = 32) {
    WPlan w;
    w.rows_per_cta = round_up(ceil_div(M, target_ctas), quantum);
    if (w.rows_per_cta < quantum) w.rows_per_cta = quantum;
    w.splits = (int)ceil_div(M, w.rows_per_cta);
    if (w.splits < 1) w.splits = 1;
    return w;
}
constexpr int kFcSplits = 8;

static size_t wgrad_tma_bytes(int64_t M, int xcols, int ycols) {
    return (size_t)wgrad_plan(M, kFcSplits, 64).splits * xcols * round_up(ycols, 64 * kFcWgradYChunks) * sizeof(float);
}
static int launch_wgrad_tma(const void* X, int xcols, const void* Y, int ycols, int64_t M, float* ws, cudaStream_t s,
                            const char* what) {
    if (xcols % (64 * kFcWgradXChunks) != 0) return fail(B200RL_ERR_INVALID_ARGUMENT, "%s: X columns must be a multiple of 128", what);
    const WPlan pl = wgrad_plan(M, kFcSplits, 64);
    CUtensorMap tmX, tmY;
    int rc;
    if ((rc = make_tmap_2d(&tmX, X, M, xcols, 64, what))) return rc;
    if ((rc = make_tmap_2d(&tmY, Y, M, ycols, 64, what))) return rc;
    const size_t smem = (size_t)4 * (kFcWgradXChunks + kFcWgradYChunks) * 64 * 128 + 1024;
    static SmemAttrCache attr;
    if ((rc = attr.ensure(tc_wgrad_tma, smem, what))) return rc;
    const dim3 grid(pl.splits, xcols / (64 * kFcWgradXChunks), (unsigned)ceil_div(ycols, 64 * kFcWgradYChunks));
    tc_wgrad_tma<<<grid, kWgradTmaThreads, smem, s>>>(tmX, tmY, M, pl.rows_per_cta, ws);
    if ((rc = check_launch(what))) return rc;
    return pl.splits;
}

}
```

cleanrl_b200/csrc/tc_heads.cuh:

```cuda
#pragma once
#include "tc_base.cuh"
#include "tc_reduce.cuh"

namespace b200rl {
using namespace tc;

constexpr int kMaxHeads = 24;
constexpr int kHeadsPartialBlocks = 264;
static inline int64_t heads_rows_per_block(int64_t n) {
    int64_t rpb = (n + kHeadsPartialBlocks - 1) / kHeadsPartialBlocks;
    if (rpb < 16) rpb = 16;
    if (rpb > 256) rpb = 256;
    return rpb;
}

template <int HT = 512>
__global__ void __launch_bounds__(256) tc_heads_fwd(const bf16* __restrict__ hid, const float* __restrict__ Wh,
                                                    const float* __restrict__ bh, int64_t n, int A1, int H,
                                                    float* __restrict__ out) {
    constexpr int NQ = (HT + 255) / 256;
    extern __shared__ float sW[];
    for (int i = threadIdx.x; i < A1 * HT; i += blockDim.x) sW[i] = Wh[i];
    __syncthreads();
    const int lane = threadIdx.x & 31, wpb = blockDim.x >> 5;
    for (int64_t row = (int64_t)blockIdx.x * wpb + (threadIdx.x >> 5); row < n; row += (int64_t)gridDim.x * wpb) {
        float hv[8 * NQ];
        const bf16* hp = hid + row * HT;
#pragma unroll
        for (int q = 0; q < NQ; ++q) {
            const bool own = HT % 256 == 0 || lane * 8 < HT;
            const int4 v = own ? ldg16(hp + q * 256 + lane * 8) : make_int4(0, 0, 0, 0);
            const uint32_t w[4] = {(uint32_t)v.x, (uint32_t)v.y, (uint32_t)v.z, (uint32_t)v.w};
#pragma unroll
            for (int e = 0; e < 4; ++e) {
                hv[q * 8 + 2 * e] = __uint_as_float(w[e] << 16);
                hv[q * 8 + 2 * e + 1] = __uint_as_float(w[e] & 0xFFFF0000u);
            }
        }
        float mine = 0.f;
        for (int a = 0; a < A1; ++a) {
            float s = 0.f;
#pragma unroll
            for (int q = 0; q < NQ; ++q) {
                if (HT % 256 != 0 && lane * 8 >= HT) continue;
                const float4 w0 = *reinterpret_cast<const float4*>(sW + a * HT + q * 256 + lane * 8);
                const float4 w1 = *reinterpret_cast<const float4*>(sW + a * HT + q * 256 + lane * 8 + 4);
                s = fmaf(hv[q * 8 + 0], w0.x, s); s = fmaf(hv[q * 8 + 1], w0.y, s);
                s = fmaf(hv[q * 8 + 2], w0.z, s); s = fmaf(hv[q * 8 + 3], w0.w, s);
                s = fmaf(hv[q * 8 + 4], w1.x, s); s = fmaf(hv[q * 8 + 5], w1.y, s);
                s = fmaf(hv[q * 8 + 6], w1.z, s); s = fmaf(hv[q * 8 + 7], w1.w, s);
            }
            s = warp_sum(s);
            if (lane == a) mine = s + bh[a];
        }
        if (lane < A1) out[row * A1 + lane] = mine;
    }
}
template <int HT = 512>
__global__ void __launch_bounds__(256) tc_heads_bwd_data(const float* __restrict__ dhead, const float* __restrict__ Wh,
                                                         const uint8_t* __restrict__ hid_bits, int64_t n, int A1, int H,
                                                         int skip_col, bf16* __restrict__ dhid) {
    constexpr int G = HT / 8;
    extern __shared__ float sWt[];
    for (int i = threadIdx.x; i < A1 * HT; i += blockDim.x) {
        const int a = i / HT, h = i % HT;
        sWt[a * HT + (h & 7) * G + (h >> 3)] = Wh[i];
    }
    __syncthreads();
    const int64_t total = n * G;
    for (int64_t idx = (int64_t)blockIdx.x * blockDim.x + threadIdx.x; idx < total; idx += (int64_t)gridDim.x * blockDim.x) {
        const int64_t row = idx / G;
        const int g = (int)(idx % G);
        const uint32_t m = hid_bits[idx];
        float o[8];
#pragma unroll
        for (int e = 0; e < 8; ++e) o[e] = 0.f;
        for (int a = 0; a < A1; ++a) {
            if (a == skip_col) continue;
            const float d = __ldg(dhead + row * A1 + a);
#pragma unroll
            for (int e = 0; e < 8; ++e) o[e] = fmaf(d, sWt[a * HT + e * G + g], o[e]);
        }
#pragma unroll
        for (int e = 0; e < 8; ++e) if (!((m >> e) & 1u)) o[e] = 0.f;
        int4 w;
        w.x = (int)pack_bf16x2(o[0], o[1]); w.y = (int)pack_bf16x2(o[2], o[3]);
        w.z = (int)pack_bf16x2(o[4], o[5]); w.w = (int)pack_bf16x2(o[6], o[7]);
        *reinterpret_cast<int4*>(dhid + row * HT + g * 8) = w;
    }
}
template <int MAXA, int HT = 512>
__global__ void __launch_bounds__(512) tc_heads_bwd_weight(const float* __restrict__ dhead, const bf16* __restrict__ hid,
                                                           int64_t n, int A1, int H, int64_t rows_per_block,
                                                           float* __restrict__ part) {
    extern __shared__ float sD[];
    const int hp = threadIdx.x % (HT / 2), rl = threadIdx.x / (HT / 2);
    const int64_t r0 = (int64_t)blockIdx.x * rows_per_block;
    int64_t r1 = r0 + rows_per_block;
    if (r1 > n) r1 = n;
    const int nrows = (int)(r1 > r0 ? r1 - r0 : 0);
    for (int i = threadIdx.x; i < nrows * A1; i += blockDim.x) sD[i] = dhead[r0 * A1 + i];
    __syncthreads();
    float acc0[MAXA], acc1[MAXA], bacc[MAXA];
#pragma unroll
    for (int a = 0; a < MAXA; ++a) { acc0[a] = 0.f; acc1[a] = 0.f; bacc[a] = 0.f; }
    const uint32_t* h2 = reinterpret_cast<const uint32_t*>(hid);
    int r = rl;
    for (; r + 14 < nrows; r += 16) {
        uint32_t hv[8];
#pragma unroll
        for (int u = 0; u < 8; ++u) hv[u] = __ldg(h2 + (r0 + r + 2 * u) * (HT / 2) + hp);
#pragma unroll
        for (int u = 0; u < 8; ++u) {
            const float x0 = __uint_as_float(hv[u] << 16), x1 = __uint_as_float(hv[u] & 0xFFFF0000u);
            const float* dr = sD + (r + 2 * u) * A1;
#pragma unroll
            for (int a = 0; a < MAXA; ++a) {
                if (a < A1) {
                    const float d = dr[a];
                    acc0[a] = fmaf(d, x0, acc0[a]); acc1[a] = fmaf(d, x1, acc1[a]); bacc[a] += d;
                }
            }
        }
    }
    for (; r < nrows; r += 2) {
        const uint32_t hv = __ldg(h2 + (r0 + r) * (HT / 2) + hp);
        const float x0 = __uint_as_float(hv << 16), x1 = __uint_as_float(hv & 0xFFFF0000u);
        const float* dr = sD + r * A1;
#pragma unroll
        for (int a = 0; a < MAXA; ++a) {
            if (a < A1) {
                const float d = dr[a];
                acc0[a] = fmaf(d, x0, acc0[a]); acc1[a] = fmaf(d, x1, acc1[a]); bacc[a] += d;
            }
        }
    }
    float* pb = part + ((int64_t)blockIdx.x * 2 + rl) * A1 * (H + 2);
#pragma unroll
    for (int a = 0; a < MAXA; ++a) {
        if (a < A1) {
            *reinterpret_cast<float2*>(pb + (int64_t)a * (H + 2) + 2 * hp) = make_float2(acc0[a], acc1[a]);
            if (hp == 0) pb[(int64_t)a * (H + 2) + H] = bacc[a];
        }
    }
}
static __global__ void __launch_bounds__(256) tc_heads_fold(const float* __restrict__ part, int nslabs, int A1, int H,
                                                     float* __restrict__ dW, float* __restrict__ db) {
    __shared__ float red[256];
    const int idx = blockIdx.x * 32 + (threadIdx.x & 31);
    const int a = idx / (H + 2), h = idx - a * (H + 2);
    const bool valid = a < A1 && h <= H;
    const float s = zlane_sum(part, (int64_t)A1 * (H + 2), nslabs, idx, valid, red);
    if (!valid || threadIdx.x >= 32) return;
    if (h == H) db[a] = s; else dW[(int64_t)a * H + h] = s;
}

template <int H>
static int heads_fwd(const bf16* hid, const float* Wh, const float* bh, int64_t n, int A1, float* out, cudaStream_t s,
                     const char* what) {
    static_assert(H == 128 || H == 256 || H == 512, "head input width");
    const int grid = (int)(ceil_div(n, 8) < (int64_t)num_sms() * 8 ? ceil_div(n, 8) : (int64_t)num_sms() * 8);
    tc_heads_fwd<H><<<grid, 256, (size_t)A1 * H * sizeof(float), s>>>(hid, Wh, bh, n, A1, H, out);
    return check_launch(what);
}
static size_t heads_partial_bytes(int64_t n, int A1, int H) {
    return (size_t)2 * ceil_div(n, heads_rows_per_block(n)) * A1 * (H + 2) * sizeof(float);
}
template <int H>
static int heads_bwd_weight(const float* dhead, const bf16* hid, int64_t n, int A1, float* part, float* dW, float* db,
                            cudaStream_t s, const char* what) {
    static_assert(H == 128 || H == 256 || H == 512, "head input width");
    const int64_t rpb = heads_rows_per_block(n);
    const int nb = (int)ceil_div(n, rpb);
    const size_t sd = (size_t)rpb * A1 * sizeof(float);
    if (A1 <= 8) tc_heads_bwd_weight<8, H><<<nb, H, sd, s>>>(dhead, hid, n, A1, H, rpb, part);
    else tc_heads_bwd_weight<kMaxHeads, H><<<nb, H, sd, s>>>(dhead, hid, n, A1, H, rpb, part);
    tc_heads_fold<<<(unsigned)ceil_div(A1 * (H + 2), 32), 256, 0, s>>>(part, 2 * nb, A1, H, dW, db);
    return check_launch(what, 2);
}
template <int H>
static int heads_bwd_data(const float* dhead, const float* Wh, const uint8_t* hid_bits, int64_t n, int A1, bf16* dhid,
                          cudaStream_t s, const char* what, int skip_col = -1) {
    static_assert(H == 128 || H == 256 || H == 512, "head input width");
    const int grid = (int)(ceil_div(n * H, 2048) < (int64_t)num_sms() * 8 ? ceil_div(n * H, 2048) : (int64_t)num_sms() * 8);
    tc_heads_bwd_data<H><<<grid, 256, (size_t)A1 * H * sizeof(float), s>>>(dhead, Wh, hid_bits, n, A1, H, skip_col, dhid);
    return check_launch(what);
}

}
```

cleanrl_b200/ops.py:

```python
from __future__ import annotations

import math

import torch

from . import _lib

STAT_NAMES = ("pg_loss", "v_loss", "entropy", "old_approx_kl", "approx_kl", "clipfrac", "loss",
              "adv_mean", "adv_std")


def _stream():
    return torch.cuda.current_stream().cuda_stream


def _ptr(t, dtype=None, name="tensor", allow_none=False):
    if t is None:
        if allow_none:
            return None
        raise ValueError(f"{name} is None")
    if not isinstance(t, torch.Tensor) or not t.is_cuda:
        raise RuntimeError(f"{name}: libb200rl kernels need a CUDA tensor (got {type(t).__name__} on "
                           f"{getattr(t, 'device', '?')}); there is no CPU fallback")
    if dtype is not None and t.dtype != dtype:
# ... 370 lines not shown
    n, C, H, W = x.shape
    y = torch.empty(n, C, (H + 1) // 2, (W + 1) // 2, dtype=torch.float32, device=x.device)
    arg = torch.empty(y.shape, dtype=torch.uint8, device=x.device)
    _lib.check(lib.b200rl_maxpool3s2_fwd_f32(_ptr(x, torch.float32, "x"), n * C, H, W, _ptr(y, torch.float32, "y"),
                                             _ptr(arg, torch.uint8, "argmax"), _stream()), "maxpool_fwd")
    return y, arg


def maxpool3s2_bwd(dy, arg, in_hw):
    lib = _lib.load()
    _contig(dy, "dy")
    n, C = dy.shape[:2]
    H, W = in_hw
    dx = torch.empty(n, C, H, W, dtype=torch.float32, device=dy.device)
    _lib.check(lib.b200rl_maxpool3s2_bwd_f32(_ptr(dy, torch.float32, "dy"), _ptr(arg, torch.uint8, "argmax"), n * C, H, W,
                                             _ptr(dx, torch.float32, "dx"), _stream()), "maxpool_bwd")
    return dx


def relu(x):
    lib = _lib.load()
    y = torch.empty_like(_contig(x, "x"))
    _lib.check(lib.b200rl_relu_f32(_ptr(x, torch.float32, "x"), x.numel(), _ptr(y, torch.float32, "y"), _stream()), "relu")
    return y


def relu_bwd(dy, x, extra=None):
    lib = _lib.load()
    dx = torch.empty_like(_contig(dy, "dy"))
    _lib.check(lib.b200rl_relu_bwd_f32(_ptr(dy, torch.float32, "dy"), _ptr(_contig(x, "x"), torch.float32, "x"),
                                       _ptr(extra, torch.float32, "extra", True), dy.numel(), _ptr(dx, torch.float32, "dx"),
                                       _stream()), "relu_bwd")
    return dx


def add(a, b):
    lib = _lib.load()
    y = torch.empty_like(_contig(a, "a"))
    _lib.check(lib.b200rl_add_f32(_ptr(a, torch.float32, "a"), _ptr(_contig(b, "b"), torch.float32, "b"), a.numel(),
                                  _ptr(y, torch.float32, "y"), _stream()), "add")
    return y


def nhwc_to_nchw_u8(x, rows=None):
    lib = _lib.load()
    _contig(x, "x")
    H, W, C = x.shape[-3:]
    n = rows.numel() if rows is not None else x.shape[0]
    y = torch.empty(n, C, H, W, dtype=torch.uint8, device=x.device)
    _lib.check(lib.b200rl_nhwc_to_nchw_u8(_ptr(x, torch.uint8, "x"), _ptr(rows, torch.int64, "rows", True), n, H, W, C,
                                          _ptr(y, torch.uint8, "y"), _stream()), "nhwc_to_nchw")
    return y


def lstm_mask_state(h, c, done, out=None):
    lib = _lib.load()
    n, H = h.shape
    f = torch.float32
    hm, cm = out if out is not None else (torch.empty_like(h), torch.empty_like(c))
    rc = lib.b200rl_lstm_mask_state_f32(_ptr(_contig(h, "h"), f, "h"), _ptr(_contig(c, "c"), f, "c"),
                                        _ptr(_contig(done, "done"), f, "done"), n, H, _ptr(hm, f, "hm"), _ptr(cm, f, "cm"), _stream())
    _lib.check(rc, "lstm_mask_state")
    return hm, cm


def lstm_cell_fwd(gates_x, gates_h, c_masked, h_out, c_out, save=None):
    lib = _lib.load()
    n, H = c_masked.shape
    f = torch.float32
    for nm, t in (("gates_x", gates_x), ("gates_h", gates_h), ("c_masked", c_masked), ("h_out", h_out), ("c_out", c_out)):
        _contig(t, nm)
    assert gates_x.shape == (n, 4 * H) and gates_h.shape == (n, 4 * H)
    rc = lib.b200rl_lstm_cell_fwd_f32(_ptr(gates_x, f, "gates_x"), _ptr(gates_h, f, "gates_h"), _ptr(c_masked, f, "c_masked"), n, H,
                                      _ptr(h_out, f, "h_out"), _ptr(c_out, f, "c_out"), _ptr(save, f, "save", True), _stream())
    _lib.check(rc, "lstm_cell_fwd")


def lstm_cell_bwd(dh_heads, dh_rec_raw, done_next, dc_rec, save, c_masked, done, dgates, dc_rec_out):
    lib = _lib.load()
    n, H = c_masked.shape
    f = torch.float32
    for nm, t in (("dh_heads", dh_heads), ("save", save), ("c_masked", c_masked), ("done", done), ("dgates", dgates),
                  ("dc_rec_out", dc_rec_out)):
        _contig(t, nm)
    rc = lib.b200rl_lstm_cell_bwd_f32(_ptr(dh_heads, f, "dh_heads"), _ptr(dh_rec_raw, f, "dh_rec_raw", True),
                                      _ptr(done_next, f, "done_next", True), _ptr(dc_rec, f, "dc_rec", True), _ptr(save, f, "save"),
                                      _ptr(c_masked, f, "c_masked"), _ptr(done, f, "done"), n, H, _ptr(dgates, f, "dgates"),
                                      _ptr(dc_rec_out, f, "dc_rec_out"), _stream())
    _lib.check(rc, "lstm_cell_bwd")


class _TensorCorePlan:

    NET = NAME = None
    MAX_A = 23
    MAX_UNPINNED = 4

    def __init__(self, A, device):
        self.A, self.device = int(A), device
        nbytes = self._c("packed_bytes")(self.A)
        if nbytes == 0:
            raise ValueError(f"{self.NAME} supports 1 <= A <= {self.MAX_A} actions (got {A})")
        self.param_count = getattr(_lib.load(), f"b200rl_{self.NET}_param_count")(self.A)
        self.packed = torch.empty(nbytes, dtype=torch.uint8, device=device)
        self._acts = {}
        self._pinned = set()
        self._ws = None
        self._pinned_ws = []

    def _c(self, name):
        return getattr(_lib.load(), f"b200rl_{self.NET}_bf16_{name}")

    def pin(self):
        self._pinned.update(self._acts)
        if self._ws is not None and all(w is not self._ws for w in self._pinned_ws):
            self._pinned_ws.append(self._ws)

    def acts(self, *shape):
        key = tuple(int(d) for d in shape)
        buf = self._acts.pop(key, None)
        if buf is None:
            unpinned = [k for k in self._acts if k not in self._pinned]
            while len(unpinned) >= self.MAX_UNPINNED:
                del self._acts[unpinned.pop(0)]
            nbytes = self._c("acts_bytes")(*key)
            if nbytes == 0:
                raise ValueError(f"{self.NAME}: batch shape {key} is out of range")
            buf = torch.zeros(nbytes, dtype=torch.uint8, device=self.device)
        self._acts[key] = buf
        return buf

    def _named_views(self, shape, specs):
        import ctypes
        off = (ctypes.c_int64 * len(specs))()
        _lib.check(self._c("acts_layout")(*shape, off), f"{self.NET}_acts_layout")
        buf = self.acts(*shape)
        return {name: buf[o:o + math.prod(dims) * dtype.itemsize].view(dtype).view(*dims)
                for o, (name, dtype, dims) in zip(off, specs) if o >= 0}

    def workspace(self, *shape):
        nbytes = self._c("workspace_bytes")(*shape, self.A)
        if self._ws is None or self._ws.numel() < nbytes:
            self._ws = torch.empty(nbytes, dtype=torch.uint8, device=self.device)
        return self._ws

    def pack(self, flat_params):
        rc = self._c("pack")(_ptr(flat_params, torch.float32, "params"), self.A, self.packed.data_ptr(), _stream())
        _lib.check(rc, f"{self.NET}_bf16_pack")


class NatureCNNBf16(_TensorCorePlan):

    NET, NAME, MAX_A = "naturecnn", "tensor-core NatureCNN", 2047

    @staticmethod
    def obs_format(obs):
        if obs.dtype == torch.uint8 and obs.dim() >= 4 and tuple(obs.shape[-3:]) == (4, 84, 84):
            return 0
        if obs.dtype == torch.bfloat16 and tuple(obs.shape[-3:]) == (21, 21, 64):
            return 1
        if obs.dtype == torch.uint8 and tuple(obs.shape[-2:]) == (441, 64):
            return 2
        raise TypeError("tensor-core NatureCNN path consumes uint8 [*,4,84,84] frames, uint8 space-to-depth rollout rows "
                        f"[*,441,64] or space-to-depth bf16 [*,21,21,64] (got {obs.dtype} {tuple(obs.shape)})")

    def forward(self, obs, rows, flat_params, head_out=None):
        lib = _lib.load()
        fmt = self.obs_format(obs)
        _contig(obs, "obs")
        n = rows.numel() if rows is not None else obs.shape[0]
        if head_out is None:
            head_out = torch.empty(n, self.A + 1, dtype=torch.float32, device=self.device)
        rc = lib.b200rl_naturecnn_bf16_forward(_ptr(obs, None, "obs"), fmt, _ptr(rows, torch.int64, "rows", True), n, self.A,
                                               _ptr(flat_params, torch.float32, "params"), self.packed.data_ptr(),
                                               self.acts(n, fmt).data_ptr(), _ptr(head_out, torch.float32, "head_out"), _stream())
        _lib.check(rc, "naturecnn_bf16_forward")
        return head_out

    def grad_tail_offset(self):
        return int(_lib.load().b200rl_naturecnn_grad_tail_offset(self.A))

    def backward(self, obs, rows, flat_params, dhead, flat_grads, tail_event=None, obs_aux=None):
        lib = _lib.load()
        fmt = self.obs_format(obs)
        if fmt == 2:
            if obs_aux is None or obs_aux.dtype != torch.uint8 or tuple(obs_aux.shape[-2:]) != (64, 448) or \
                    obs_aux.shape[0] != obs.shape[0]:
                raise ValueError("uint8 rollout rows need their channel-major copy [*,64,448] (obs_aux) for the backward pass")
            _contig(obs_aux, "obs_aux")
        n = dhead.shape[0]
        _contig(dhead, "dhead")
        ws = self.workspace(n)
        rc = lib.b200rl_naturecnn_bf16_backward(_ptr(obs, None, "obs"), _ptr(obs_aux, None, "obs_aux", True), fmt,
                                                _ptr(rows, torch.int64, "rows", True), n, self.A,
                                                _ptr(flat_params, torch.float32, "params"), self.packed.data_ptr(),
                                                self.acts(n, fmt).data_ptr(), _ptr(dhead, torch.float32, "dhead"),
                                                _ptr(flat_grads, torch.float32, "grads"), ws.data_ptr(), ws.numel(),
                                                tail_event.cuda_event if tail_event is not None else None, _stream())
        _lib.check(rc, "naturecnn_bf16_backward")


class ImpalaCNNBf16(_TensorCorePlan):

    NET, NAME = "impala", "tensor-core IMPALA-CNN"
    VALUE_HEADS = 1

    def act_tensors(self, n):
        bf, u8, i32 = torch.bfloat16, torch.uint8, torch.int32
        specs = [("c0", bf, (n, 64, 64, 16)), ("c1", bf, (n, 32, 32, 32)), ("c2", bf, (n, 16, 16, 32))]
        for q, shp in enumerate(((n, 32, 32, 16), (n, 16, 16, 32), (n, 8, 8, 32))):
            specs += [(f"{name}_{q}", bf, shp) for name in ("s0", "s1", "s2", "y0", "y1")] + [(f"arg_{q}", u8, shp)]
        specs += [("h0", bf, (n, 2048)), ("mh0", i32, (n, 64)), ("hid", bf, (n, 256)), ("mhid", i32, (n, 8)),
                  ("dc", bf, (n, 65536)), ("ga", bf, (n, 16384)), ("gb", bf, (n, 16384)), ("gy", bf, (n, 16384)),
                  ("dhid", bf, (n, 256))]
        return self._named_views((n,), specs)

    @staticmethod
    def check_obs(obs):
        if obs.dtype != torch.uint8 or obs.dim() < 4 or tuple(obs.shape[-3:]) != (64, 64, 3):
            raise ValueError("tensor-core IMPALA-CNN consumes uint8 frames [*, 64, 64, 3] "
                             f"(got {obs.dtype} {tuple(obs.shape)})")

    def forward(self, obs, rows, flat_params, head_out=None):
        self.check_obs(obs)
        _contig(obs, "obs")
        n = rows.numel() if rows is not None else obs.shape[0]
        if rows is not None:
            _contig(rows, "rows")
        if head_out is None:
            head_out = torch.empty(n, self.A + self.VALUE_HEADS, dtype=torch.float32, device=self.device)
        rc = self._c("forward")(_ptr(obs, torch.uint8, "obs"), _ptr(rows, torch.int64, "rows", True), n,
                                self.A, _ptr(flat_params, torch.float32, "params"), self.packed.data_ptr(),
                                self.acts(n).data_ptr(), _ptr(head_out, torch.float32, "head_out"), _stream())
        _lib.check(rc, f"{self.NET}_bf16_forward")
        return head_out

    def backward(self, obs, rows, flat_params, dhead, flat_grads):
        self.check_obs(obs)
        _contig(dhead, "dhead")
        n = dhead.shape[0]
        ws = self.workspace(n)
        rc = self._c("backward")(_ptr(obs, torch.uint8, "obs"), _ptr(rows, torch.int64, "rows", True), n,
                                 self.A, _ptr(flat_params, torch.float32, "params"), self.packed.data_ptr(),
                                 self.acts(n).data_ptr(), _ptr(dhead, torch.float32, "dhead"),
                                 _ptr(flat_grads, torch.float32, "grads"), ws.data_ptr(), ws.numel(), _stream())
        _lib.check(rc, f"{self.NET}_bf16_backward")


class ImpalaPPGBf16(ImpalaCNNBf16):

    NET, NAME, MAX_A, VALUE_HEADS = "impala_ppg", "tensor-core IMPALA-CNN (PPG heads)", 22, 2

    def _c(self, name):
        return super()._c(name) if not name.startswith("acts_") else getattr(_lib.load(), f"b200rl_impala_bf16_{name}")


class LSTMAgentBf16(_TensorCorePlan):

    NET, NAME = "lstm_agent", "tensor-core LSTM agent"
    H = 128

    def act_tensors(self, S, n):
        M = S * n
        bf, f32, i32 = torch.bfloat16, torch.float32, torch.int32
        return self._named_views((S, n), [
            ("act1", bf, (M, 10, 10, 128)), ("m1", i32, (M, 400)), ("act2", bf, (M, 9, 9, 64)), ("act3", bf, (M, 7, 7, 64)),
            ("feats", bf, (M, 512)), ("m4", i32, (M, 16)),
            ("gx", f32, (M, 512)), ("hseq", bf, (M, 128)), ("hm", bf, (M, 128)), ("save", f32, (M, 5, 128)),
            ("cm", f32, (M, 128)), ("dgates", f32, (M, 512)), ("dfeats", bf, (M, 512))])

    @staticmethod
    def check_obs(obs):
        if obs.dtype != torch.uint8 or obs.dim() != 4 or tuple(obs.shape[-3:]) != (1, 84, 84):
            raise ValueError("tensor-core LSTM agent consumes uint8 frames [*, 1, 84, 84] "
                             f"(got {obs.dtype} {tuple(obs.shape)})")

    def forward(self, obs, rows, S, n, flat_params, h0, c0, done, head_out=None, h_out=None, c_out=None):
        self.check_obs(obs)
        _contig(obs, "obs")
        f = torch.float32
        M = S * n
        if rows is not None:
            _contig(rows, "rows")
            if rows.numel() != M:
                raise ValueError(f"rows has {rows.numel()} entries for {S} steps x {n} envs")
        elif obs.shape[0] != M:
            raise ValueError(f"obs has {obs.shape[0]} frames for {S} steps x {n} envs")
        for nm, t, shape in (("h0", h0, (n, self.H)), ("c0", c0, (n, self.H)), ("done", done, (M,))):
            _contig(t, nm)
            if tuple(t.shape) != shape:
                raise ValueError(f"{nm}: expected shape {shape}, got {tuple(t.shape)}")
        if head_out is None:
            head_out = torch.empty(M, self.A + 1, dtype=f, device=self.device)
        if h_out is None:
            h_out = torch.empty(n, self.H, dtype=f, device=self.device)
        if c_out is None:
            c_out = torch.empty(n, self.H, dtype=f, device=self.device)
        rc = _lib.load().b200rl_lstm_agent_bf16_forward(
            _ptr(obs, torch.uint8, "obs"), _ptr(rows, torch.int64, "rows", True), S, n, self.A,
            _ptr(flat_params, f, "params"), self.packed.data_ptr(), _ptr(h0, f, "h0"), _ptr(c0, f, "c0"),
            _ptr(done, f, "done"), self.acts(S, n).data_ptr(), _ptr(head_out, f, "head_out"), _ptr(h_out, f, "h_out"),
            _ptr(c_out, f, "c_out"), _stream())
        _lib.check(rc, "lstm_agent_bf16_forward")
        return head_out, h_out, c_out

    def backward(self, obs, rows, S, n, flat_params, done, dhead, flat_grads):
        self.check_obs(obs)
        _contig(dhead, "dhead")
        ws = self.workspace(S, n)
        f = torch.float32
        rc = _lib.load().b200rl_lstm_agent_bf16_backward(
            _ptr(obs, torch.uint8, "obs"), _ptr(rows, torch.int64, "rows", True), S, n, self.A,
            _ptr(flat_params, f, "params"), self.packed.data_ptr(), _ptr(done, f, "done"), self.acts(S, n).data_ptr(),
            _ptr(dhead, f, "dhead"), _ptr(flat_grads, f, "grads"), ws.data_ptr(), ws.numel(), _stream())
        _lib.check(rc, "lstm_agent_bf16_backward")


def frames_to_s2d(obs_u8, out=None, rows=None):
    lib = _lib.load()
    _contig(obs_u8, "obs")
    n = rows.numel() if rows is not None else obs_u8.shape[0]
    if out is None:
        out = torch.empty(n, 21, 21, 64, dtype=torch.bfloat16, device=obs_u8.device)
    rc = lib.b200rl_frames_to_s2d_bf16(_ptr(obs_u8, torch.uint8, "obs"), _ptr(rows, torch.int64, "rows", True), n,
                                       _ptr(out, torch.bfloat16, "out"), _stream())
    _lib.check(rc, "frames_to_s2d")
    return out


def alloc_u8_rollout_rows(shape, device):
# ... 262 lines not shown
```

include/b200rl.h:

```cpp
#ifndef B200RL_H
#define B200RL_H

#include <stddef.h>
#include <stdint.h>

#ifdef __cplusplus
extern "C" {
#endif

typedef enum {
    B200RL_OK = 0,
    B200RL_ERR_INVALID_ARGUMENT = -1,
    B200RL_ERR_CUDA = -2,
    B200RL_ERR_UNSUPPORTED = -3,
    B200RL_ERR_WORKSPACE = -4
} b200rl_status;

int b200rl_version(void);
const char* b200rl_last_error(void);
int b200rl_compiled_arch(void);

long long b200rl_launch_count(void);
void b200rl_profile_enable(int on);
void b200rl_profile_reset(void);
int b200rl_profile_summary(char* buf, size_t capacity);

int b200rl_gae_f32(const float* rewards, const float* values, const float* dones,
                   const float* next_value, const float* next_done,
                   float* advantages, float* returns,
                   int64_t T, int64_t N, double gamma, double gae_lambda,
                   int mode, void* stream);

int b200rl_categorical_sample_f32(const float* logits, int64_t ld_logits, const float* noise,
                                  const float* value_in, int64_t ld_value,
                                  int64_t n, int A,
                                  int64_t* action, float* logprob, float* entropy, float* value_out,
                                  void* stream);

int b200rl_categorical_eval_f32(const float* logits, int64_t ld_logits, const int64_t* action,
                                int64_t n, int A, float* logprob, float* entropy, void* stream);

size_t b200rl_ppo_loss_workspace_bytes(int64_t M);
int b200rl_ppo_loss_f32(const float* new_logits, int64_t ld_logits,
                        const float* new_value, int64_t ld_value,
                        const int64_t* mb_inds,
                        const int64_t* b_actions, const float* b_logprobs,
                        const float* b_advantages, const float* b_returns, const float* b_values,
                        int64_t M, int A,
                        double clip_coef, double ent_coef, double vf_coef,
                        int norm_adv, int clip_vloss,
                        float* dlogits, int64_t ld_dlogits, float* dvalue, int64_t ld_dvalue,
                        float* stats, void* workspace, size_t workspace_bytes, void* stream);

int b200rl_gaussian_sample_f32(const float* mean, int64_t ld_mean, const float* logstd, const float* noise,
                               const float* value_in, int64_t ld_value, int64_t n, int D,
                               float* action, float* logprob, float* entropy, float* value_out, void* stream);
int b200rl_gaussian_eval_f32(const float* mean, int64_t ld_mean, const float* logstd, const float* action,
                             int64_t n, int D, float* logprob, float* entropy, void* stream);
size_t b200rl_ppo_loss_gaussian_workspace_bytes(int64_t M);
int b200rl_ppo_loss_gaussian_f32(const float* new_mean, int64_t ld_mean, const float* logstd,
                                 const float* new_value, int64_t ld_value, const int64_t* mb_inds,
                                 const float* b_actions, const float* b_logprobs,
                                 const float* b_advantages, const float* b_returns, const float* b_values,
                                 int64_t M, int D, double clip_coef, double ent_coef, double vf_coef,
                                 int norm_adv, int clip_vloss,
                                 float* dmean, int64_t ld_dmean, float* dlogstd, float* dvalue, int64_t ld_dvalue,
                                 float* stats, void* workspace, size_t workspace_bytes, void* stream);

size_t b200rl_clip_adam_workspace_bytes(int64_t P);
int b200rl_clip_adam_f32(float* params, const float* grads, float* exp_avg, float* exp_avg_sq,
                         int64_t P, int64_t step, double lr, double beta1, double beta2, double eps,
                         double max_norm, int world_size, float* norm_out,
                         void* workspace, size_t workspace_bytes, void* stream);
int b200rl_adam_step_scalars(int64_t step, double lr, double beta1, double beta2, float* out2);
int b200rl_clip_adam_dyn_f32(float* params, const float* grads, float* exp_avg, float* exp_avg_sq,
                             int64_t P, const float* step_scalars, double beta1, double beta2, double eps,
                             double max_norm, int world_size, float* norm_out,
                             void* workspace, size_t workspace_bytes, void* stream);

int b200rl_clip_adam_ranges_f32(float* params, const float* grads, float* exp_avg, float* exp_avg_sq, int64_t P,
                                int64_t step, double lr, const int64_t* ranges, int nranges, int64_t range_step,
                                double range_lr, double beta1, double beta2, double eps, double max_norm,
                                float* norm_out, void* workspace, size_t workspace_bytes, void* stream);
int b200rl_clip_adam_ranges_dyn_f32(float* params, const float* grads, float* exp_avg, float* exp_avg_sq, int64_t P,
                                    const float* step_scalars, const int64_t* ranges, int nranges, int frozen,
                                    double beta1, double beta2, double eps, double max_norm, float* norm_out,
                                    void* workspace, size_t workspace_bytes, void* stream);

size_t b200rl_ppg_aux_loss_workspace_bytes(int64_t n);
int b200rl_ppg_aux_loss_f32(const float* head_out, int64_t ld_head, const int64_t* rows, const float* old_logits,
                            const float* returns, int64_t n, int A, double beta_clone, double inv_accum,
                            float* dhead, int64_t ld_dhead, float* stats, void* workspace, size_t workspace_bytes,
                            void* stream);

enum { B200RL_ACT_NONE = 0, B200RL_ACT_RELU = 1, B200RL_ACT_TANH = 2 };
enum { B200RL_DT_F32 = 0, B200RL_DT_U8 = 1 };

int b200rl_conv2d_fwd_f32(const void* x, int x_dtype, const int64_t* rows, double in_div,
                          const float* w, const float* b, float* y,
                          int64_t n, int Cin, int H, int W, int Cout, int KH, int KW, int stride,
                          int act, void* stream);
int b200rl_conv2d_fwd_pad_f32(const void* x, int x_dtype, const int64_t* rows, double in_div,
                              const float* w, const float* b, float* y,
                              int64_t n, int Cin, int H, int W, int Cout, int KH, int KW, int stride, int pad,
                              int act, void* stream);
int b200rl_conv2d_bwd_data_pad_f32(const float* dy, const float* w, const float* x_post, int prev_act, float* dx,
                                   int64_t n, int Cin, int H, int W, int Cout, int KH, int KW, int stride, int pad, void* stream);
size_t b200rl_conv2d_bwd_weight_pad_workspace_bytes(int64_t n, int Cin, int H, int W, int Cout, int KH, int KW, int stride, int pad);
int b200rl_conv2d_bwd_weight_pad_f32(const void* x, int x_dtype, const int64_t* rows, double in_div,
                                     const float* dy, float* dw, float* db,
                                     int64_t n, int Cin, int H, int W, int Cout, int KH, int KW, int stride, int pad,
                                     void* workspace, size_t workspace_bytes, void* stream);
int b200rl_maxpool3s2_fwd_f32(const float* x, int64_t nc, int H, int W, float* y, uint8_t* argmax, void* stream);
int b200rl_maxpool3s2_bwd_f32(const float* dy, const uint8_t* argmax, int64_t nc, int H, int W, float* dx, void* stream);
int b200rl_relu_f32(const float* x, int64_t n, float* y, void* stream);
int b200rl_relu_bwd_f32(const float* dy, const float* x, const float* extra, int64_t n, float* dx, void* stream);
int b200rl_add_f32(const float* a, const float* b, int64_t n, float* y, void* stream);
int b200rl_nhwc_to_nchw_u8(const uint8_t* x, const int64_t* rows, int64_t n, int H, int W, int C, uint8_t* y, void* stream);
int b200rl_conv2d_bwd_data_f32(const float* dy, const float* w, const float* x_post, int prev_act,
                               float* dx,
                               int64_t n, int Cin, int H, int W, int Cout, int KH, int KW, int stride,
                               void* stream);
size_t b200rl_conv2d_bwd_weight_workspace_bytes(int64_t n, int Cin, int H, int W, int Cout, int KH, int KW, int stride);
int b200rl_conv2d_bwd_weight_f32(const void* x, int x_dtype, const int64_t* rows, double in_div,
                                 const float* dy, float* dw, float* db,
                                 int64_t n, int Cin, int H, int W, int Cout, int KH, int KW, int stride,
                                 void* workspace, size_t workspace_bytes, void* stream);
int b200rl_linear_fwd_f32(const float* x, const int64_t* rows, const float* w, const float* b, float* y,
                          int64_t n, int in_features, int out_features, int act, void* stream);
int b200rl_linear_bwd_data_f32(const float* dy, const float* w, const float* x_post, int prev_act, float* dx,
                               int64_t n, int in_features, int out_features, void* stream);
size_t b200rl_linear_bwd_weight_workspace_bytes(int64_t n, int in_features, int out_features);
int b200rl_linear_bwd_weight_f32(const float* x, const int64_t* rows, const float* dy, float* dw, float* db,
                                 int64_t n, int in_features, int out_features,
                                 void* workspace, size_t workspace_bytes, void* stream);

enum { B200RL_OBS_U8_NCHW = 0, B200RL_OBS_S2D_BF16 = 1, B200RL_OBS_S2D_U8 = 2 };
int b200rl_frames_to_s2d_bf16(const uint8_t* obs, const int64_t* rows, int64_t n, void* out_s2d, void* stream);
int b200rl_frames_to_s2d_u8(const uint8_t* obs, const int64_t* rows, int64_t n, uint8_t* out_rm, uint8_t* out_cm, void* stream);
int b200rl_frames_delta_s2d_u8(const uint8_t* new_planes, const int32_t* full_slot, const uint8_t* full_frames,
                               const uint8_t* prev_rm, const uint8_t* prev_cm, int64_t n,
                               uint8_t* out_rm, uint8_t* out_cm, void* stream);
int b200rl_h2d_rows_async(void* dst, const void* src, int64_t src_pitch, int64_t row_bytes, int64_t rows, void* stream);
void* b200rl_stackdelta_create(int64_t n_envs, int planes, int64_t plane_bytes, int threads);
void b200rl_stackdelta_destroy(void* tracker);
void b200rl_stackdelta_invalidate(void* tracker);
int64_t b200rl_stackdelta_begin(void* tracker, const uint8_t* obs, int64_t env_stride, const float* done,
                                uint8_t* new_out, uint8_t* full_out, int32_t* slot_out);
int64_t b200rl_stackdelta_wait(void* tracker, int32_t* mismatch_out);
typedef struct B200rlPartLaunch {
    void* tracker;
    void* copy_stream;
    void* main_stream;
    void* consumed_event;
    int32_t n, nchunks;
    int32_t chunk_lo[4], chunk_hi[4];
    void* h2d_event[4];
    void* graph_exec[4];
    uint8_t* new_d; int32_t* slot_d; uint8_t* full_d;
    uint8_t* new_h; uint8_t* full_h; int32_t* slot_h;
    const void* actions_d; void* actions_h; int64_t actions_bytes; void* d2h_event;
} B200rlPartLaunch;
int b200rl_mt19937_shuffle_i64(uint32_t* key624, int32_t* pos, int64_t* data, int64_t n);
int64_t b200rl_stackdelta_launch(const B200rlPartLaunch* plan, const uint8_t* obs, int64_t env_stride, const float* done);
int64_t b200rl_stackdelta_join(void* tracker, void* d2h_event, int32_t* mismatch_out);
int64_t b200rl_naturecnn_param_count(int A);
size_t b200rl_naturecnn_bf16_packed_bytes(int A);
size_t b200rl_naturecnn_bf16_acts_bytes(int64_t n, int obs_format);
size_t b200rl_naturecnn_bf16_workspace_bytes(int64_t n, int A);
int b200rl_naturecnn_bf16_pack(const float* params, int A, void* packed, void* stream);
int b200rl_naturecnn_bf16_forward(const void* obs, int obs_format, const int64_t* rows, int64_t n, int A,
                                  const float* params, const void* packed, void* acts,
                                  float* head_out, void* stream);
int b200rl_naturecnn_bf16_backward(const void* obs, const void* obs_aux, int obs_format, const int64_t* rows, int64_t n, int A,
                                   const float* params, const void* packed, void* acts,
                                   const float* dhead, float* grads,
                                   void* workspace, size_t workspace_bytes, void* tail_ready_event, void* stream);
int64_t b200rl_naturecnn_grad_tail_offset(int A);

int64_t b200rl_impala_param_count(int A);
size_t b200rl_impala_bf16_packed_bytes(int A);
size_t b200rl_impala_bf16_acts_bytes(int64_t n);
#define B200RL_IMPALA_ACTS_TENSORS 30
int b200rl_impala_bf16_acts_layout(int64_t n, int64_t* offsets);
size_t b200rl_impala_bf16_workspace_bytes(int64_t n, int A);
int b200rl_impala_bf16_pack(const float* params, int A, void* packed, void* stream);
int b200rl_impala_bf16_forward(const uint8_t* obs, const int64_t* rows, int64_t n, int A, const float* params,
                               const void* packed, void* acts, float* head_out, void* stream);
int b200rl_impala_bf16_backward(const uint8_t* obs, const int64_t* rows, int64_t n, int A, const float* params,
                                const void* packed, void* acts, const float* dhead, float* grads,
                                void* workspace, size_t workspace_bytes, void* stream);

int64_t b200rl_impala_ppg_param_count(int A);
size_t b200rl_impala_ppg_bf16_packed_bytes(int A);
size_t b200rl_impala_ppg_bf16_workspace_bytes(int64_t n, int A);
int b200rl_impala_ppg_bf16_pack(const float* params, int A, void* packed, void* stream);
int b200rl_impala_ppg_bf16_forward(const uint8_t* obs, const int64_t* rows, int64_t n, int A, const float* params,
                                   const void* packed, void* acts, float* head_out, void* stream);
int b200rl_impala_ppg_bf16_backward(const uint8_t* obs, const int64_t* rows, int64_t n, int A, const float* params,
                                    const void* packed, void* acts, const float* dhead, float* grads,
                                    void* workspace, size_t workspace_bytes, void* stream);

int64_t b200rl_lstm_agent_param_count(int A);
size_t b200rl_lstm_agent_bf16_packed_bytes(int A);
size_t b200rl_lstm_agent_bf16_acts_bytes(int64_t S, int64_t n);
#define B200RL_LSTM_ACTS_TENSORS 13
int b200rl_lstm_agent_bf16_acts_layout(int64_t S, int64_t n, int64_t* offsets);
size_t b200rl_lstm_agent_bf16_workspace_bytes(int64_t S, int64_t n, int A);
int b200rl_lstm_agent_bf16_pack(const float* params, int A, void* packed, void* stream);
int b200rl_lstm_agent_bf16_forward(const uint8_t* obs, const int64_t* rows, int64_t S, int64_t n, int A,
                                   const float* params, const void* packed, const float* h0, const float* c0,
                                   const float* done, void* acts, float* head_out, float* h_out, float* c_out, void* stream);
int b200rl_lstm_agent_bf16_backward(const uint8_t* obs, const int64_t* rows, int64_t S, int64_t n, int A,
                                    const float* params, const void* packed, const float* done, void* acts,
                                    const float* dhead, float* grads, void* workspace, size_t workspace_bytes, void* stream);

int b200rl_lstm_mask_state_f32(const float* h, const float* c, const float* done, int64_t n, int H,
                               float* h_masked, float* c_masked, void* stream);
int b200rl_lstm_cell_fwd_f32(const float* gates_x, const float* gates_h, const float* c_masked, int64_t n, int H,
                             float* h_out, float* c_out, float* save, void* stream);
int b200rl_lstm_cell_bwd_f32(const float* dh_heads, const float* dh_rec_raw, const float* done_next, const float* dc_rec,
                             const float* save, const float* c_masked, const float* done, int64_t n, int H,
                             float* dgates, float* dc_rec_out, void* stream);

size_t b200rl_dqn_td_loss_workspace_bytes(int64_t B);
int b200rl_dqn_td_loss_f32(const float* q, int64_t ld_q, const float* q_target_next, int64_t ld_qt,
                           const int64_t* actions, const float* rewards, const float* dones,
                           int64_t B, int A, double gamma, int huber,
                           float* dq, int64_t ld_dq, float* stats,
                           void* workspace, size_t workspace_bytes, void* stream);
int b200rl_argmax_f32(const float* q, int64_t ld_q, int64_t n, int A, int64_t* out, void* stream);

int b200rl_c51_act_f32(const float* logits, int64_t ld, const float* atoms, int64_t n, int A, int n_atoms,
                       const int64_t* action_in, int64_t* action_out, float* q_out, float* pmf_out, void* stream);
size_t b200rl_c51_loss_workspace_bytes(int64_t B);
int b200rl_c51_loss_f32(const float* logits, int64_t ld, const float* next_logits, int64_t ld_next,
                        const float* atoms, const int64_t* actions, const float* rewards, const float* dones,
                        int64_t B, int A, int n_atoms, double gamma, double v_min, double v_max,
                        float* dlogits, int64_t ld_d, float* stats,
                        void* workspace, size_t workspace_bytes, void* stream);

#ifdef __cplusplus
}
#endif
#endif
```

Before: 1.193 million.

## Fuse rollout policy heads with categorical sampling and retile small-batch FC GEMM

Adds a fused NatureCNN policy_step entry point. Its heads kernel computes logits and value and also draws the categorical sample, logprob and value in the same kernel, so the separate sampling launch and the logits round-trip through memory go away during rollout. It also adds a 64-row M tile variant of the TMA GEMM for the FC layer when the batch is small enough to leave SMs idle. Separately, it rewrites the frame-to-space-to-depth kernel to process a whole frame per block, using byte_perm transposes. These changes add code paths and a new tile configuration, and the fused path only applies to the bf16 uint8 s2d observation layout with a small action count.

```diff
diff --git a/cleanrl_b200/_lib.py b/cleanrl_b200/_lib.py
--- a/cleanrl_b200/_lib.py
+++ b/cleanrl_b200/_lib.py
@@ -66,6 +66,7 @@
     "b200rl_naturecnn_bf16_workspace_bytes": (_sz, [_i64, _i]),
     "b200rl_naturecnn_bf16_pack": (_i, [_p, _i, _p, _p]),
     "b200rl_naturecnn_bf16_forward": (_i, [_p, _i, _p, _i64, _i, _p, _p, _p, _p, _p]),
+    "b200rl_naturecnn_bf16_policy_step": (_i, [_p, _i64, _i, _p, _p, _p, _p, _p, _p, _p, _p]),
     "b200rl_naturecnn_bf16_backward": (_i, [_p, _p, _i, _p, _i64, _i, _p, _p, _p, _p, _p, _p, _sz, _p, _p]),
     "b200rl_frames_to_s2d_u8": (_i, [_p, _p, _i64, _p, _p, _p]),
     "b200rl_lstm_mask_state_f32": (_i, [_p, _p, _p, _i64, _i, _p, _p, _p]),
diff --git a/cleanrl_b200/agents.py b/cleanrl_b200/agents.py
--- a/cleanrl_b200/agents.py
+++ b/cleanrl_b200/agents.py
@@ -226,6 +226,15 @@
             self._hidden = hidden
         A = self.num_actions
         return out[:, :A], out[:, A]
+
+    def sample_into(self, obs, actions_out, logprobs_out, values_out, noise=None):
+        A = self.num_actions
+        if not (self.precision == "bf16" and obs.dtype == torch.uint8 and tuple(obs.shape[-2:]) == (441, 64)
+                and A + 1 <= ops.NatureCNNBf16.MAX_NARROW_HEADS):
+            return super().sample_into(obs, actions_out, logprobs_out, values_out, noise=noise)
+        tc = self._tc_plan()
+        q = noise if noise is not None else self.noise_fn(obs.shape[0], A, obs.device)
+        tc.policy_step(obs, self._flat.flat, q, actions_out, logprobs_out, values_out)
 
     def forward_train(self, b_obs, mb_inds, aux=None):
         self.flat
diff --git a/cleanrl_b200/csrc/categorical.cuh b/cleanrl_b200/csrc/categorical.cuh
--- /dev/null
+++ b/cleanrl_b200/csrc/categorical.cuh
@@ -0,0 +1,54 @@
+#pragma once
+#include <cfloat>
+#include "common.cuh"
+
+namespace b200rl {
+
+struct RowStats {
+    float lse;
+    float m2;
+    float s2;
+};
+
+__device__ __forceinline__ RowStats row_stats(const float* __restrict__ x, int A) {
+    float m = -INFINITY;
+    for (int k = 0; k < A; ++k) m = fmaxf(m, x[k]);
+    const float mm = (fabsf(m) == INFINITY) ? 0.f : m;
+    float s = 0.f;
+    for (int k = 0; k < A; ++k) s += expf(x[k] - mm);
+    RowStats r;
+    r.lse = logf(s) + mm;
+    float m2 = -INFINITY;
+    for (int k = 0; k < A; ++k) m2 = fmaxf(m2, x[k] - r.lse);
+    float s2 = 0.f;
+    for (int k = 0; k < A; ++k) s2 += expf((x[k] - r.lse) - m2);
+    r.m2 = m2;
+    r.s2 = s2;
+    return r;
+}
+
+struct RowSample {
+    int action;
+    float logprob;
+    float entropy;
+};
+
+__device__ __forceinline__ RowSample categorical_sample_row(const float* __restrict__ x, const float* __restrict__ q, int A) {
+    const RowStats rs = row_stats(x, A);
+    float best = -INFINITY, ent = 0.f;
+    int arg = 0;
+    for (int k = 0; k < A; ++k) {
+        const float nl = x[k] - rs.lse;
+        const float p = expf(nl - rs.m2) / rs.s2;
+        const float sc = p / q[k];
+        if (sc > best) { best = sc; arg = k; }
+        ent += fmaxf(nl, -FLT_MAX) * p;
+    }
+    RowSample r;
+    r.action = arg;
+    r.logprob = x[arg] - rs.lse;
+    r.entropy = -ent;
+    return r;
+}
+
+}
diff --git a/cleanrl_b200/csrc/net_tc.cu b/cleanrl_b200/csrc/net_tc.cu
--- a/cleanrl_b200/csrc/net_tc.cu
+++ b/cleanrl_b200/csrc/net_tc.cu
@@ -192,7 +192,8 @@
     p.Bw = P + L.wfcf; p.N = 512; p.out = act + Q.hid; p.ldo = 512; p.bias = params + L.fcb; p.relu = 1;
     p.mask_out = reinterpret_cast<uint32_t*>(act + Q.m4);
     { ProfScope ps(s, "fc_fwd", 2.0 * n * 512 * 3136, (double)n * (3136 + 512) * 2 + 512.0 * 3136 * 2);
-      if (n <= 8192) { if ((rc = launch_gemm_tma<64, 6>(p, s, "naturecnn/fc"))) return rc; }
+      if (ceil_div(n, 128) * (512 / 64) <= num_sms() / 2) { if ((rc = launch_gemm_tma<64, 8, 64>(p, s, "naturecnn/fc"))) return rc; }
+      else if (n <= 8192) { if ((rc = launch_gemm_tma<64, 6>(p, s, "naturecnn/fc"))) return rc; }
       else if ((rc = launch_gemm_tma<128, 4>(p, s, "naturecnn/fc"))) return rc; }
     return B200RL_OK;
 }
@@ -343,7 +344,7 @@
     B200RL_REQUIRE(n <= (int64_t)1 << 28, "frames_to_s2d_u8: n too large");
     cudaStream_t s = (cudaStream_t)stream;
     ProfScope ps(s, "frames_to_s2d", 0, (double)n * (28224 + 28224 + 28672));
-    tc_frames_to_s2d_u8<<<(unsigned)(n * 4), 256, 0, s>>>(obs, rows, n, out_rm, out_cm);
+    tc_frames_to_s2d_u8<<<(unsigned)n, kS2dThreads, 0, s>>>(obs, rows, n, out_rm, out_cm);
     return check_launch("frames_to_s2d_u8");
 }
 
@@ -380,6 +381,19 @@
         return check_launch("naturecnn_pack", 7);
     }
     return check_launch("naturecnn_pack", 6);
+}
+
+namespace b200rl {
+static int conv1_u8_fwd(const NatureLayout& L, const NatureActs& Q, const float* params, const bf16* P, const void* obs,
+                        const int64_t* rows, int64_t n, bf16* act, cudaStream_t s) {
+    Conv1U8Params cp;
+    memset(&cp, 0, sizeof(cp));
+    cp.rows = rows; cp.n = (int)n; cp.n_images = rows ? (int64_t)1 << 24 : n;
+    cp.limbs = reinterpret_cast<const int8_t*>(P + L.w1l); cp.sc = reinterpret_cast<const float*>(P + L.w1sc);
+    cp.bias = params + L.c1b; cp.out = act + Q.act1; cp.mask_out = reinterpret_cast<uint32_t*>(act + Q.m1);
+    ProfScope ps(s, "conv1_fwd", 2.0 * n * 400 * 32 * 256, (double)n * (28224 + 12800 * 2 + 1600));
+    return launch_conv1_i8(cp, obs, s, "naturecnn/conv1_i8");
+}
 }
 
 extern "C" int b200rl_naturecnn_bf16_forward(const void* obs, int obs_format, const int64_t* rows, int64_t n, int A,
@@ -407,13 +421,7 @@
         x0 = act + Q.x0; x0rows = nullptr;
     }
     if (obs_format == B200RL_OBS_S2D_U8) {
-        Conv1U8Params cp;
-        memset(&cp, 0, sizeof(cp));
-        cp.rows = rows; cp.n = (int)n; cp.n_images = rows ? (int64_t)1 << 24 : n;
-        cp.limbs = reinterpret_cast<const int8_t*>(P + L.w1l); cp.sc = reinterpret_cast<const float*>(P + L.w1sc);
-        cp.bias = params + L.c1b; cp.out = act + Q.act1; cp.mask_out = reinterpret_cast<uint32_t*>(act + Q.m1);
-        ProfScope ps(s, "conv1_fwd", 2.0 * n * 400 * 32 * 256, (double)n * (28224 + 12800 * 2 + 1600));
-        if ((rc = launch_conv1_i8(cp, obs, s, "naturecnn/conv1_i8"))) return rc;
+        if ((rc = conv1_u8_fwd(L, Q, params, P, obs, rows, n, act, s))) return rc;
     } else {
     win_defaults(wp); win_conv1(wp, x0, x0rows, n);
     wp.Bw = P + L.w1f; wp.N = 32; wp.vH = 20; wp.vW = 20; wp.out_mode = WOUT_S2D2; wp.out = act + Q.act1;
@@ -428,6 +436,30 @@
     }
     ProfScope ps(s, "heads_fwd", 2.0 * n * 512 * (A + 1), (double)n * (1024 + 4 * (A + 1)));
     return heads_fwd<512>(act + Q.hid, params + L.hw, params + L.hb, n, A + 1, head_out, s, "naturecnn/heads");
+}
+
+extern "C" int b200rl_naturecnn_bf16_policy_step(const uint8_t* obs_s2d, int64_t n, int A, const float* params,
+                                                 const void* packed, void* acts, const float* noise, int64_t* actions,
+                                                 float* logprobs, float* values, void* stream) {
+    B200RL_REQUIRE(n >= 0, "naturecnn_policy_step: negative n");
+    if (n == 0) return B200RL_OK;
+    B200RL_REQUIRE(obs_s2d && params && packed && acts && noise && actions && logprobs && values,
+                   "naturecnn_policy_step: null pointer");
+    B200RL_REQUIRE(A >= 1 && A + 1 <= kMaxHeads, "naturecnn_policy_step: A=%d outside [1,%d]", A, kMaxHeads - 1);
+    B200RL_REQUIRE(aligned(obs_s2d, 16) && aligned(acts, 16) && aligned(packed, 16) && aligned(noise, 4) && aligned(actions, 8) &&
+                   aligned(logprobs, 4) && aligned(values, 4), "naturecnn_policy_step: misaligned buffer");
+    B200RL_REQUIRE(n <= (int64_t)1 << 22, "naturecnn_policy_step: n too large");
+    const NatureLayout L(A);
+    const NatureActs Q(n, false);
+    const bf16* P = reinterpret_cast<const bf16*>(packed);
+    bf16* act = reinterpret_cast<bf16*>(acts);
+    cudaStream_t s = (cudaStream_t)stream;
+    int rc;
+    if ((rc = conv1_u8_fwd(L, Q, params, P, obs_s2d, nullptr, n, act, s))) return rc;
+    if ((rc = trunk_fwd(L, Q, params, P, act, n, s))) return rc;
+    ProfScope ps(s, "heads_sample", 2.0 * n * 512 * (A + 1), (double)n * (1024 + 4 * A + 16));
+    return heads_sample<512>(act + Q.hid, params + L.hw, params + L.hb, n, A + 1, noise, actions, logprobs, values, s,
+                             "naturecnn/heads_sample");
 }
 
 extern "C" int b200rl_naturecnn_bf16_backward(const void* obs, const void* obs_aux, int obs_format, const int64_t* rows, int64_t n, int A,
diff --git a/cleanrl_b200/csrc/policy.cu b/cleanrl_b200/csrc/policy.cu
--- a/cleanrl_b200/csrc/policy.cu
+++ b/cleanrl_b200/csrc/policy.cu
@@ -1,32 +1,10 @@
 #include "common.cuh"
+#include "categorical.cuh"
 #include <cfloat>
 
 namespace b200rl {
 
 constexpr int kMaxA = 64;
-
-struct RowStats {
-    float lse;
-    float m2;
-    float s2;
-};
-
-__device__ __forceinline__ RowStats row_stats(const float* __restrict__ x, int A) {
-    float m = -INFINITY;
-    for (int k = 0; k < A; ++k) m = fmaxf(m, x[k]);
-    const float mm = (fabsf(m) == INFINITY) ? 0.f : m;
-    float s = 0.f;
-    for (int k = 0; k < A; ++k) s += expf(x[k] - mm);
-    RowStats r;
-    r.lse = logf(s) + mm;
-    float m2 = -INFINITY;
-    for (int k = 0; k < A; ++k) m2 = fmaxf(m2, x[k] - r.lse);
-    float s2 = 0.f;
-    for (int k = 0; k < A; ++k) s2 += expf((x[k] - r.lse) - m2);
-    r.m2 = m2;
-    r.s2 = s2;
-    return r;
-}
 
 __global__ void __launch_bounds__(128) categorical_sample_kernel(
     const float* __restrict__ logits, int64_t ld, const float* __restrict__ noise,
@@ -35,21 +13,10 @@
     float* __restrict__ value_out) {
     const int64_t i = (int64_t)blockIdx.x * blockDim.x + threadIdx.x;
     if (i >= n) return;
-    const float* x = logits + i * ld;
-    const float* q = noise + i * (int64_t)A;
-    const RowStats rs = row_stats(x, A);
-    float best = -INFINITY, ent = 0.f;
-    int arg = 0;
-    for (int k = 0; k < A; ++k) {
-        const float nl = x[k] - rs.lse;
-        const float p = expf(nl - rs.m2) / rs.s2;
-        const float sc = p / q[k];
-        if (sc > best) { best = sc; arg = k; }
-        ent += fmaxf(nl, -FLT_MAX) * p;
-    }
-    action[i] = arg;
-    logprob[i] = x[arg] - rs.lse;
-    if (entropy) entropy[i] = -ent;
+    const RowSample r = categorical_sample_row(logits + i * ld, noise + i * (int64_t)A, A);
+    action[i] = r.action;
+    logprob[i] = r.logprob;
+    if (entropy) entropy[i] = r.entropy;
     if (value_out && value_in) value_out[i] = value_in[i * ldv];
 }
 
diff --git a/cleanrl_b200/csrc/tc_conv1_u8.cuh b/cleanrl_b200/csrc/tc_conv1_u8.cuh
--- a/cleanrl_b200/csrc/tc_conv1_u8.cuh
+++ b/cleanrl_b200/csrc/tc_conv1_u8.cuh
@@ -13,36 +13,55 @@
     return (uint64_t)((smem_addr & 0x3FFFFu) >> 4) | ((uint64_t)((lbo >> 4) & 0x3FFF) << 16) | (32ull << 32) | kDescSwizzle64;
 }
 __device__ __forceinline__ uint32_t img64_off(int r, int c) { return (uint32_t)(r * 64 + ((c ^ ((r >> 1) & 3)) << 4)); }
-__global__ void __launch_bounds__(256) tc_frames_to_s2d_u8(const uint8_t* __restrict__ obs, const int64_t* __restrict__ rows, int64_t n,
-                                                           uint8_t* __restrict__ out_rm, uint8_t* __restrict__ out_cm) {
-    __shared__ __align__(16) uint8_t plane[7056];
-    const int64_t i = blockIdx.x >> 2;
-    const int c = blockIdx.x & 3;
+constexpr int kS2dThreads = 448;
+__global__ void __launch_bounds__(kS2dThreads) tc_frames_to_s2d_u8(const uint8_t* __restrict__ obs, const int64_t* __restrict__ rows,
+                                                                   int64_t n, uint8_t* __restrict__ out_rm, uint8_t* __restrict__ out_cm) {
+    constexpr int kChunks = 28224 / 16;
+    constexpr int kPer = (kChunks + kS2dThreads - 1) / kS2dThreads;
+    __shared__ __align__(16) uint8_t frame[28224];
+    const int64_t i = blockIdx.x;
     const int64_t img = rows ? rows[i] : i;
-    const int4* src = reinterpret_cast<const int4*>(obs + img * 28224 + c * 7056);
-    for (int t = threadIdx.x; t < 441; t += 256) reinterpret_cast<int4*>(plane)[t] = __ldg(src + t);
+    const int4* src = reinterpret_cast<const int4*>(obs + img * 28224);
+    int4 v[kPer];
+#pragma unroll
+    for (int k = 0; k < kPer; ++k) {
+        const int t = threadIdx.x + k * kS2dThreads;
+        if (t < kChunks) v[k] = __ldg(src + t);
+    }
+#pragma unroll
+    for (int k = 0; k < kPer; ++k) {
+        const int t = threadIdx.x + k * kS2dThreads;
+        if (t < kChunks) reinterpret_cast<int4*>(frame)[t] = v[k];
+    }
     __syncthreads();
-    for (int pos = threadIdx.x; pos < 441; pos += 256) {
+    int4* rm = reinterpret_cast<int4*>(out_rm + i * 28224);
+    for (int t = threadIdx.x; t < kChunks; t += kS2dThreads) {
+        const int pos = t >> 2, c = t & 3;
         const int Y = pos / 21, X = pos - Y * 21;
-        const uint8_t* p = plane + (Y * 4) * 84 + X * 4;
-        int4 v;
-        v.x = *reinterpret_cast<const int*>(p); v.y = *reinterpret_cast<const int*>(p + 84);
-        v.z = *reinterpret_cast<const int*>(p + 168); v.w = *reinterpret_cast<const int*>(p + 252);
-        *reinterpret_cast<int4*>(out_rm + (i * 441 + pos) * 64 + c * 16) = v;
-    }
-    for (int t = threadIdx.x; t < 16 * 112; t += 256) {
-        const int ch = t / 112, q = t - ch * 112;
-        const int sy = ch >> 2, sx = ch & 3;
-        uint32_t w = 0;
+        const uint8_t* p = frame + c * 7056 + (Y * 4) * 84 + X * 4;
+        int4 w;
+        w.x = *reinterpret_cast<const int*>(p); w.y = *reinterpret_cast<const int*>(p + 84);
+        w.z = *reinterpret_cast<const int*>(p + 168); w.w = *reinterpret_cast<const int*>(p + 252);
+        rm[t] = w;
+    }
+    uint32_t* cm = reinterpret_cast<uint32_t*>(out_cm + i * 28672);
+    for (int t = threadIdx.x; t < 16 * 112; t += kS2dThreads) {
+        const int cs = t / 112, q = t - cs * 112;
+        const uint8_t* pl = frame + (cs >> 2) * 7056 + (cs & 3) * 84;
+        uint32_t w[4];
 #pragma unroll
         for (int e = 0; e < 4; ++e) {
             const int pos = q * 4 + e;
-            if (pos < 441) {
-                const int Y = pos / 21, X = pos - Y * 21;
-                w |= (uint32_t)plane[(Y * 4 + sy) * 84 + X * 4 + sx] << (8 * e);
-            }
-        }
-        *reinterpret_cast<uint32_t*>(out_cm + (i * 64 + c * 16 + ch) * 448 + q * 4) = w;
+            const int Y = pos / 21, X = pos - Y * 21;
+            w[e] = pos < 441 ? *reinterpret_cast<const uint32_t*>(pl + Y * 336 + X * 4) : 0u;
+        }
+        const uint32_t lo01 = __byte_perm(w[0], w[1], 0x5140), hi01 = __byte_perm(w[0], w[1], 0x7362);
+        const uint32_t lo23 = __byte_perm(w[2], w[3], 0x5140), hi23 = __byte_perm(w[2], w[3], 0x7362);
+        uint32_t* dst = cm + cs * 4 * 112 + q;
+        dst[0] = __byte_perm(lo01, lo23, 0x5410);
+        dst[112] = __byte_perm(lo01, lo23, 0x7632);
+        dst[224] = __byte_perm(hi01, hi23, 0x5410);
+        dst[336] = __byte_perm(hi01, hi23, 0x7632);
     }
 }
 
diff --git a/cleanrl_b200/csrc/tc_gemm_tma.cuh b/cleanrl_b200/csrc/tc_gemm_tma.cuh
--- a/cleanrl_b200/csrc/tc_gemm_tma.cuh
+++ b/cleanrl_b200/csrc/tc_gemm_tma.cuh
@@ -26,14 +26,16 @@
 constexpr int kGemmThreads = 384;
 template <int BN>
 __host__ __device__ constexpr size_t gemm_acc_bytes() { return (size_t)128 * (BN + 4) * sizeof(float); }
-template <int BN, int STAGES>
+template <int BN, int STAGES, int BM = 128>
 __global__ void __launch_bounds__(kGemmThreads, 1) tc_gemm_tma(const __grid_constant__ CUtensorMap tmA,
                                                                const __grid_constant__ CUtensorMap tmB,
                                                                const KGemmParams p, int total_tiles, int ntiles_n) {
-    constexpr int A_BYTES = 128 * 128;
+    static_assert(BM == 128 || BM == 64, "tile rows");
+    constexpr int WN = BM == 128 ? BN : BN / 2;
+    constexpr int A_BYTES = BM * 128;
     constexpr int B_BYTES = BN * 128;
     constexpr int STAGE_BYTES = A_BYTES + B_BYTES;
-    constexpr int LDA = BN + 4;
+    constexpr int LDA = WN + 4;
     extern __shared__ uint8_t smem_raw[];
     __shared__ uint64_t full_bar[STAGES], empty_bar[STAGES];
     uint8_t* smem = reinterpret_cast<uint8_t*>((reinterpret_cast<uintptr_t>(smem_raw) + 1023) & ~uintptr_t(1023));
@@ -58,7 +60,7 @@
                     if (q >= (uint32_t)STAGES) mbar_wait(&empty_bar[s], ((q / STAGES) - 1) & 1);
                     const uint32_t dst = smem_u32(smem + (size_t)s * STAGE_BYTES);
                     mbar_arrive_expect_tx(&full_bar[s], STAGE_BYTES);
-                    tma_load_2d(dst, &tmA, j * 64, mt * 128, &full_bar[s]);
+                    tma_load_2d(dst, &tmA, j * 64, mt * BM, &full_bar[s]);
                     tma_load_2d(dst + A_BYTES, &tmB, j * 64, n0, &full_bar[s]);
                 }
             }
@@ -68,27 +70,28 @@
         float* st = sAcc + wg * 64 * LDA;
         const int lr = wt & 63, half = wt >> 6;
         const int nwords = p.N >> 5;
-        constexpr int NW = BN / 32;
-        float d[BN / 2];
-#pragma unroll
-        for (int e = 0; e < BN / 2; ++e) d[e] = 0.f;
+        constexpr int NW = WN / 32;
+        float d[WN / 2];
+#pragma unroll
+        for (int e = 0; e < WN / 2; ++e) d[e] = 0.f;
         uint32_t q = 0;
         for (int tile = blockIdx.x; tile < total_tiles; tile += gridDim.x) {
-            const int mt = tile / ntiles_n, n0 = (tile - mt * ntiles_n) * BN;
+            const int mt = tile / ntiles_n, n0 = (tile - mt * ntiles_n) * BN + (BM == 128 ? 0 : wg * WN);
             for (int j = 0; j < nch; ++j, ++q) {
                 const uint32_t s = q % STAGES;
                 mbar_wait(&full_bar[s], (q / STAGES) & 1);
                 wgmma_fence();
                 const uint32_t stage_addr = smem_u32(smem + (size_t)s * STAGE_BYTES);
-                const uint64_t a = desc_kmajor(stage_addr + wg * 64 * 128), b = desc_kmajor(stage_addr + A_BYTES);
-#pragma unroll
-                for (int kk = 0; kk < 4; ++kk) WgmmaBf16<BN, 0, 0>::mma(d, a + 2 * kk, b + 2 * kk, (j | kk) != 0 ? 1u : 0u);
+                const uint64_t a = desc_kmajor(stage_addr + (BM == 128 ? wg * 64 * 128 : 0)),
+                               b = desc_kmajor(stage_addr + A_BYTES + (BM == 128 ? 0 : wg * WN * 128));
+#pragma unroll
+                for (int kk = 0; kk < 4; ++kk) WgmmaBf16<WN, 0, 0>::mma(d, a + 2 * kk, b + 2 * kk, (j | kk) != 0 ? 1u : 0u);
                 wgmma_commit();
                 wgmma_wait<0>();
                 mbar_arrive(&empty_bar[s]);
             }
             wgmma_fence_operands(d);
-            const int r = mt * 128 + wg * 64 + lr;
+            const int r = mt * BM + (BM == 128 ? wg * 64 : 0) + lr;
             const bool rvalid = r < (int)p.M;
             const int64_t wb = (int64_t)r * nwords + (n0 >> 5);
             named_bar(1 + wg, 128);
@@ -234,22 +237,22 @@
     }
 }
 
-template <int BN, int STAGES>
+template <int BN, int STAGES, int BM = 128>
 static int launch_gemm_tma(const KGemmParams& p, cudaStream_t s, const char* what) {
-    const size_t smem = (size_t)STAGES * (128 * 128 + BN * 128) + gemm_acc_bytes<BN>() + 1024;
+    const size_t smem = (size_t)STAGES * (BM * 128 + BN * 128) + gemm_acc_bytes<BN>() + 1024;
     static SmemAttrCache attr;
     int rc;
     if (p.N % 64 != 0 || BN % 64 != 0) return fail(B200RL_ERR_INVALID_ARGUMENT, "%s: N must be a multiple of 64", what);
-    if ((rc = attr.ensure(tc_gemm_tma<BN, STAGES>, smem, what))) return rc;
+    if ((rc = attr.ensure(tc_gemm_tma<BN, STAGES, BM>, smem, what))) return rc;
     CUtensorMap tmA, tmB;
     const int64_t K = (int64_t)p.nchunks * 64;
-    if ((rc = make_tmap_2d(&tmA, p.A, p.M, K, 128, what))) return rc;
+    if ((rc = make_tmap_2d(&tmA, p.A, p.M, K, BM, what))) return rc;
     if ((rc = make_tmap_2d(&tmB, p.Bw, p.N, K, BN, what))) return rc;
     const int ntn = (int)ceil_div(p.N, BN);
-    const int total = (int)ceil_div(p.M, 128) * ntn;
+    const int total = (int)ceil_div(p.M, BM) * ntn;
     int grid = num_sms();
     if (grid > total) grid = total;
-    tc_gemm_tma<BN, STAGES><<<grid, kGemmThreads, smem, s>>>(tmA, tmB, p, total, ntn);
+    tc_gemm_tma<BN, STAGES, BM><<<grid, kGemmThreads, smem, s>>>(tmA, tmB, p, total, ntn);
     return check_launch(what);
 }
 
diff --git a/cleanrl_b200/csrc/tc_heads.cuh b/cleanrl_b200/csrc/tc_heads.cuh
--- a/cleanrl_b200/csrc/tc_heads.cuh
+++ b/cleanrl_b200/csrc/tc_heads.cuh
@@ -1,6 +1,7 @@
 #pragma once
 #include "tc_base.cuh"
 #include "tc_reduce.cuh"
+#include "categorical.cuh"
 
 namespace b200rl {
 using namespace tc;
@@ -14,46 +15,92 @@
     return rpb;
 }
 
+template <int HT>
+__device__ __forceinline__ void head_load(const bf16* __restrict__ hp, int lane, float (&hv)[8 * ((HT + 255) / 256)]) {
+    constexpr int NQ = (HT + 255) / 256;
+#pragma unroll
+    for (int q = 0; q < NQ; ++q) {
+        const bool own = HT % 256 == 0 || lane * 8 < HT;
+        const int4 v = own ? ldg16(hp + q * 256 + lane * 8) : make_int4(0, 0, 0, 0);
+        const uint32_t w[4] = {(uint32_t)v.x, (uint32_t)v.y, (uint32_t)v.z, (uint32_t)v.w};
+#pragma unroll
+        for (int e = 0; e < 4; ++e) {
+            hv[q * 8 + 2 * e] = __uint_as_float(w[e] << 16);
+            hv[q * 8 + 2 * e + 1] = __uint_as_float(w[e] & 0xFFFF0000u);
+        }
+    }
+}
+template <int HT>
+__device__ __forceinline__ float head_dot(const float (&hv)[8 * ((HT + 255) / 256)], const float* sW, const float* __restrict__ bh,
+                                          int A1, int lane) {
+    constexpr int NQ = (HT + 255) / 256;
+    float mine = 0.f;
+    for (int a = 0; a < A1; ++a) {
+        float s = 0.f;
+#pragma unroll
+        for (int q = 0; q < NQ; ++q) {
+            if (HT % 256 != 0 && lane * 8 >= HT) continue;
+            const float4 w0 = *reinterpret_cast<const float4*>(sW + a * HT + q * 256 + lane * 8);
+            const float4 w1 = *reinterpret_cast<const float4*>(sW + a * HT + q * 256 + lane * 8 + 4);
+            s = fmaf(hv[q * 8 + 0], w0.x, s); s = fmaf(hv[q * 8 + 1], w0.y, s);
+            s = fmaf(hv[q * 8 + 2], w0.z, s); s = fmaf(hv[q * 8 + 3], w0.w, s);
+            s = fmaf(hv[q * 8 + 4], w1.x, s); s = fmaf(hv[q * 8 + 5], w1.y, s);
+            s = fmaf(hv[q * 8 + 6], w1.z, s); s = fmaf(hv[q * 8 + 7], w1.w, s);
+        }
+        s = warp_sum(s);
+        if (lane == a) mine = s + bh[a];
+    }
+    return mine;
+}
+
 template <int HT = 512>
 __global__ void __launch_bounds__(256) tc_heads_fwd(const bf16* __restrict__ hid, const float* __restrict__ Wh,
                                                     const float* __restrict__ bh, int64_t n, int A1, int H,
                                                     float* __restrict__ out) {
-    constexpr int NQ = (HT + 255) / 256;
     extern __shared__ float sW[];
     for (int i = threadIdx.x; i < A1 * HT; i += blockDim.x) sW[i] = Wh[i];
     __syncthreads();
     const int lane = threadIdx.x & 31, wpb = blockDim.x >> 5;
     for (int64_t row = (int64_t)blockIdx.x * wpb + (threadIdx.x >> 5); row < n; row += (int64_t)gridDim.x * wpb) {
-        float hv[8 * NQ];
-        const bf16* hp = hid + row * HT;
-#pragma unroll
-        for (int q = 0; q < NQ; ++q) {
-            const bool own = HT % 256 == 0 || lane * 8 < HT;
-            const int4 v = own ? ldg16(hp + q * 256 + lane * 8) : make_int4(0, 0, 0, 0);
-            const uint32_t w[4] = {(uint32_t)v.x, (uint32_t)v.y, (uint32_t)v.z, (uint32_t)v.w};
-#pragma unroll
-            for (int e = 0; e < 4; ++e) {
-                hv[q * 8 + 2 * e] = __uint_as_float(w[e] << 16);
-                hv[q * 8 + 2 * e + 1] = __uint_as_float(w[e] & 0xFFFF0000u);
-            }
-        }
-        float mine = 0.f;
-        for (int a = 0; a < A1; ++a) {
-            float s = 0.f;
-#pragma unroll
-            for (int q = 0; q < NQ; ++q) {
-                if (HT % 256 != 0 && lane * 8 >= HT) continue;
-                const float4 w0 = *reinterpret_cast<const float4*>(sW + a * HT + q * 256 + lane * 8);
-                const float4 w1 = *reinterpret_cast<const float4*>(sW + a * HT + q * 256 + lane * 8 + 4);
-                s = fmaf(hv[q * 8 + 0], w0.x, s); s = fmaf(hv[q * 8 + 1], w0.y, s);
-                s = fmaf(hv[q * 8 + 2], w0.z, s); s = fmaf(hv[q * 8 + 3], w0.w, s);
-                s = fmaf(hv[q * 8 + 4], w1.x, s); s = fmaf(hv[q * 8 + 5], w1.y, s);
-                s = fmaf(hv[q * 8 + 6], w1.z, s); s = fmaf(hv[q * 8 + 7], w1.w, s);
-            }
-            s = warp_sum(s);
-            if (lane == a) mine = s + bh[a];
-        }
+        float hv[8 * ((HT + 255) / 256)];
+        head_load<HT>(hid + row * HT, lane, hv);
+        const float mine = head_dot<HT>(hv, sW, bh, A1, lane);
         if (lane < A1) out[row * A1 + lane] = mine;
+    }
+}
+
+template <int HT = 512>
+__global__ void __launch_bounds__(256) tc_heads_sample(const bf16* __restrict__ hid, const float* __restrict__ Wh,
+                                                       const float* __restrict__ bh, int64_t n, int A1,
+                                                       const float* __restrict__ noise, int64_t* __restrict__ action,
+                                                       float* __restrict__ logprob, float* __restrict__ value) {
+    extern __shared__ float sW[];
+    __shared__ float sOut[8][kMaxHeads];
+    const int lane = threadIdx.x & 31, w = threadIdx.x >> 5, wpb = blockDim.x >> 5;
+    const int64_t stride = (int64_t)gridDim.x * wpb;
+    int64_t row = (int64_t)blockIdx.x * wpb + w;
+    float hv[8 * ((HT + 255) / 256)];
+    if (row < n) head_load<HT>(hid + row * HT, lane, hv);
+    if ((reinterpret_cast<uintptr_t>(Wh) & 15) == 0) {
+        for (int i = threadIdx.x; i < A1 * HT / 4; i += blockDim.x)
+            reinterpret_cast<float4*>(sW)[i] = __ldg(reinterpret_cast<const float4*>(Wh) + i);
+    } else {
+        for (int i = threadIdx.x; i < A1 * HT; i += blockDim.x) sW[i] = Wh[i];
+    }
+    __syncthreads();
+    const int A = A1 - 1;
+    for (; row < n; row += stride) {
+        const float mine = head_dot<HT>(hv, sW, bh, A1, lane);
+        if (row + stride < n) head_load<HT>(hid + (row + stride) * HT, lane, hv);
+        if (lane < A1) sOut[w][lane] = mine;
+        __syncwarp();
+        if (lane == 0) {
+            const RowSample r = categorical_sample_row(sOut[w], noise + row * A, A);
+            action[row] = r.action;
+            logprob[row] = r.logprob;
+            value[row] = sOut[w][A];
+        }
+        __syncwarp();
     }
 }
 template <int HT = 512>
@@ -163,6 +210,14 @@
     tc_heads_fwd<H><<<grid, 256, (size_t)A1 * H * sizeof(float), s>>>(hid, Wh, bh, n, A1, H, out);
     return check_launch(what);
 }
+template <int H>
+static int heads_sample(const bf16* hid, const float* Wh, const float* bh, int64_t n, int A1, const float* noise,
+                        int64_t* action, float* logprob, float* value, cudaStream_t s, const char* what) {
+    static_assert(H == 128 || H == 256 || H == 512, "head input width");
+    const int grid = (int)(ceil_div(n, 8) < (int64_t)num_sms() * 8 ? ceil_div(n, 8) : (int64_t)num_sms() * 8);
+    tc_heads_sample<H><<<grid, 256, (size_t)A1 * H * sizeof(float), s>>>(hid, Wh, bh, n, A1, noise, action, logprob, value);
+    return check_launch(what);
+}
 static size_t heads_partial_bytes(int64_t n, int A1, int H) {
     return (size_t)2 * ceil_div(n, heads_rows_per_block(n)) * A1 * (H + 2) * sizeof(float);
 }
diff --git a/cleanrl_b200/ops.py b/cleanrl_b200/ops.py
--- a/cleanrl_b200/ops.py
+++ b/cleanrl_b200/ops.py
@@ -546,6 +546,7 @@
 class NatureCNNBf16(_TensorCorePlan):
 
     NET, NAME, MAX_A = "naturecnn", "tensor-core NatureCNN", 2047
+    MAX_NARROW_HEADS = 24
 
     @staticmethod
     def obs_format(obs):
@@ -570,6 +571,24 @@
                                                self.acts(n, fmt).data_ptr(), _ptr(head_out, torch.float32, "head_out"), _stream())
         _lib.check(rc, "naturecnn_bf16_forward")
         return head_out
+
+    def policy_step(self, obs, flat_params, noise, actions, logprobs, values):
+        if self.obs_format(obs) != 2:
+            raise TypeError("policy_step takes uint8 space-to-depth rollout rows [n,441,64]")
+        n = obs.shape[0]
+        _contig(obs, "obs")
+        _contig(noise, "noise")
+        if tuple(noise.shape) != (n, self.A):
+            raise ValueError(f"noise must be [{n}, {self.A}] (got {tuple(noise.shape)})")
+        for t, name in ((actions, "actions"), (logprobs, "logprobs"), (values, "values")):
+            _contig(t, name)
+            if t.numel() != n:
+                raise ValueError(f"{name} must hold {n} entries (got {t.numel()})")
+        rc = _lib.load().b200rl_naturecnn_bf16_policy_step(
+            _ptr(obs, torch.uint8, "obs"), n, self.A, _ptr(flat_params, torch.float32, "params"), self.packed.data_ptr(),
+            self.acts(n, 2).data_ptr(), _ptr(noise, torch.float32, "noise"), _ptr(actions, torch.int64, "actions"),
+            _ptr(logprobs, torch.float32, "logprobs"), _ptr(values, torch.float32, "values"), _stream())
+        _lib.check(rc, "naturecnn_bf16_policy_step")
 
     def grad_tail_offset(self):
         return int(_lib.load().b200rl_naturecnn_grad_tail_offset(self.A))
diff --git a/include/b200rl.h b/include/b200rl.h
--- a/include/b200rl.h
+++ b/include/b200rl.h
@@ -172,6 +172,9 @@
 int b200rl_naturecnn_bf16_forward(const void* obs, int obs_format, const int64_t* rows, int64_t n, int A,
                                   const float* params, const void* packed, void* acts,
                                   float* head_out, void* stream);
+int b200rl_naturecnn_bf16_policy_step(const uint8_t* obs_s2d, int64_t n, int A, const float* params, const void* packed,
+                                      void* acts, const float* noise, int64_t* actions, float* logprobs, float* values,
+                                      void* stream);
 int b200rl_naturecnn_bf16_backward(const void* obs, const void* obs_aux, int obs_format, const int64_t* rows, int64_t n, int A,
                                    const float* params, const void* packed, void* acts,
                                    const float* dhead, float* grads,
```

Measured after the change: 1.221 million (median of 6 runs). +2.3%, better.
